# alexrich021/3dvnet

Hardware: AMD Instinct MI355X
Metric: depth maps/sec (256x320, 96 planes, 7 src) (higher is better)
Workload: dtype f32 storage/accumulate; MFMA operands split-bf16x3 (hi*hi+hi*lo+lo*hi, 16 mantissa bits); warp/variance f32 VALU; 1 GPU; cfg2: ScanNet-shape 256x320, 1 ref + 7 src (8 edges/ref), 96 planes, 56x56 plane grid, 32-ch quarter features 64x80; fused warp+variance -> CostRegNet -> soft-argmin depth (rows A1-A6); n_img_per_gpu=71, edges_per_ref=8, parallelism=single GPU, launch=eager, ranks_seen=1

## Files before the change

3dvnet_amd/_lib.py:

```python
import ctypes
import os

import torch

_HERE = os.path.dirname(os.path.abspath(__file__))
LIB_PATH = os.path.join(_HERE, 'lib3dvnet_hip.so')
ABI_VERSION = 9
PRECISION = {'split_bf16': 0, 'fp32': 1}


def precision_code(name):
    try:
        return PRECISION[name]
    except KeyError:
        raise ValueError("precision must be 'split_bf16' or 'fp32', got %r" % (name,))


c_void_p, c_int, c_float, c_double, c_size_t = (ctypes.c_void_p, ctypes.c_int, ctypes.c_float,
                                                ctypes.c_double, ctypes.c_size_t)
c_float_p = ctypes.POINTER(ctypes.c_float)
c_float_pp = ctypes.POINTER(c_float_p)

SIGNATURES = {
    'v3d_version': (c_int, []),
    'v3d_last_error': (ctypes.c_char_p, []),
    'v3d_set_option': (c_int, [ctypes.c_char_p, c_int]),
    'v3d_get_option': (c_int, [ctypes.c_char_p, ctypes.POINTER(c_int)]),
    'v3d_timing_enable': (c_int, [c_int]),
    'v3d_timing_collect': (c_int, [c_int, ctypes.c_char_p, c_int, ctypes.POINTER(c_float),
                                   ctypes.POINTER(c_int)]),
    'v3d_psv_workspace_bytes': (c_size_t, [c_int] * 4),
    'v3d_psv_variance_f32': (c_int, [c_void_p] * 7 + [c_int] * 8 + [c_double] * 2 + [c_int] * 3 +
                             [c_void_p, c_void_p, c_size_t, c_void_p]),
    'v3d_psv_sample_positions_f32': (c_int, [c_void_p] * 6 + [c_int] * 7 + [c_double] * 2 + [c_int] * 3 +
                                     [c_void_p, c_void_p, c_void_p, c_size_t, c_void_p]),
    'v3d_psv_variance_split': (c_int, [c_void_p] * 7 + [c_int] * 8 + [c_double] * 2 + [c_int] * 3 +
                               [c_void_p, c_void_p, c_size_t, c_void_p]),
    'v3d_psv_variance_cl8': (c_int, [c_void_p] * 7 + [c_int] * 8 + [c_double] * 2 + [c_int] * 3 +
                             [c_void_p, c_void_p, c_size_t, c_void_p]),
    'v3d_costreg_depth_cl8': (c_int, [c_void_p] * 3 + [c_int] * 4 + [c_void_p, c_void_p, c_void_p,
                                                                    c_size_t, c_void_p]),
    'v3d_costreg_pack': (c_int, [c_float_pp] * 5 + [c_float_p, c_float_p, c_int, c_int, c_float,
                                                     ctypes.POINTER(c_void_p)]),
    'v3d_costreg_free': (None, [c_void_p]),
    'v3d_costreg_workspace_bytes': (c_size_t, [c_void_p] + [c_int] * 4),
    'v3d_costreg_depth_f32': (c_int, [c_void_p] * 3 + [c_int] * 4 + [c_void_p, c_void_p, c_int, c_void_p,
                                                                    c_size_t, c_void_p]),
    'v3d_costreg_depth_split': (c_int, [c_void_p] * 3 + [c_int] * 4 + [c_void_p, c_void_p, c_void_p,
                                                                      c_size_t, c_void_p]),
    'v3d_costreg_layer_f32': (c_int, [c_void_p, c_int, c_void_p, c_void_p] + [c_int] * 4 +
                              [c_void_p, c_int, c_void_p]),
    'v3d_costreg_layer_split_workspace_bytes': (c_size_t, [c_int] * 5),
    'v3d_costreg_layer_split_f32': (c_int, [c_void_p, c_int, c_void_p, c_void_p] + [c_int] * 4 +
                                    [c_void_p, c_void_p, c_size_t, c_void_p]),
    'v3d_propagation_pack': (c_int, [c_float_pp] * 5 + [c_int, c_int, c_float, ctypes.POINTER(c_void_p)]),
    'v3d_propagation_free': (None, [c_void_p]),
    'v3d_propagation_up_f32': (c_int, [c_void_p, c_void_p, c_void_p] + [c_int] * 6 + [c_void_p, c_void_p, c_void_p, c_int, c_void_p]),
    'v3d_backproject_workspace_bytes': (c_size_t, [c_int] * 4),
    'v3d_backproject_variance_f32': (c_int, [c_void_p] * 8 + [c_int] * 10 + [c_double, c_int] +
                                     [c_void_p, c_void_p, c_void_p, c_size_t, c_void_p]),
    'v3d_gemm_pack': (c_int, [c_float_p, ctypes.c_longlong, ctypes.c_longlong, ctypes.c_longlong,
                              c_int, c_int, c_int, c_float_p, c_float_p, c_float_p, c_float_p,
                              ctypes.POINTER(c_void_p)]),
    'v3d_gemm_free': (None, [c_void_p]),
    'v3d_gemm_gather_f32': (c_int, [c_void_p, c_int, ctypes.POINTER(c_void_p), ctypes.POINTER(c_void_p),
                                    ctypes.POINTER(c_int), c_int, c_int, c_int, c_float, c_void_p, c_int,
                                    c_int, c_void_p, c_void_p, c_int, c_void_p, c_int, c_int, c_void_p]),
    'v3d_sparse_conv_f32': (c_int, [c_void_p, c_int, c_void_p, c_int, c_void_p, ctypes.c_longlong, c_int, c_float, c_void_p,
                                    c_int, c_int, c_void_p, c_int, c_int, c_void_p]),
    'v3d_fill_f32': (c_int, [c_void_p, c_size_t, c_float, c_void_p]),
    'v3d_pointnet_input_f32': (c_int, [c_void_p] * 5 + [c_int, c_int, c_void_p, c_void_p]),
    'v3d_hash_bytes': (c_size_t, [c_int]),
    'v3d_hash_build': (c_int, [c_void_p, c_int, c_void_p, c_size_t, c_void_p]),
    'v3d_hash_status': (c_int, [c_void_p, c_int, c_void_p]),
    'v3d_sparse_neighbors': (c_int, [c_void_p, c_int, c_void_p, c_int, c_int, c_void_p, c_void_p]),
    'v3d_sparse_interp_workspace_bytes': (c_size_t, [c_int, c_int]),
    'v3d_sparse_interp_f32': (c_int, [c_void_p, c_int, c_void_p, c_int, c_int, c_void_p, c_void_p, c_int,
                                      c_int, c_void_p, c_float, c_void_p, c_int, c_int, c_void_p, c_size_t,
                                      c_void_p]),
    'v3d_edges_csr_workspace_bytes': (c_size_t, [c_int, c_int]),
    'v3d_edges_csr': (c_int, [c_void_p, c_int, c_int, c_int, c_void_p, c_void_p, c_void_p, c_void_p, c_size_t, c_void_p]),
    'v3d_edges_csr_status': (c_int, [c_void_p, c_size_t, c_void_p]),
    'v3d_segment_csr_workspace_bytes': (c_size_t, [c_int]),
    'v3d_segment_csr': (c_int, [c_void_p, c_int, c_int, c_void_p, c_void_p, c_void_p, c_size_t, c_void_p]),
    'v3d_segment_max_f32': (c_int, [c_void_p, c_int, c_void_p, c_void_p, c_int, c_int, c_void_p, c_int, c_void_p]),
    'v3d_sort_unique_workspace_bytes': (c_size_t, [c_int]),
    'v3d_sort_unique_u64': (c_int, [c_void_p, c_int, c_void_p, ctypes.POINTER(c_int), c_void_p, c_size_t, c_void_p]),
    'v3d_strided_keys': (c_int, [c_void_p, c_int, c_int, c_void_p, c_void_p]),
    'v3d_unpack_coords': (c_int, [c_void_p, c_int, c_void_p, c_void_p]),
    'v3d_voxelize_workspace_bytes': (c_size_t, []),
    'v3d_voxel_keys': (c_int, [c_void_p, c_void_p, c_int, c_float, c_void_p, c_void_p, c_size_t, c_void_p]),
    'v3d_voxelize_status': (c_int, [c_void_p, c_size_t, c_void_p]),
    'v3d_lower_bound_u64': (c_int, [c_void_p, c_int, c_void_p, c_int, c_void_p, c_void_p]),
    'v3d_voxel_decode': (c_int, [c_void_p, c_int, c_float, c_float, c_void_p, c_void_p, c_void_p, c_void_p,
                                 c_size_t, c_void_p]),
    'v3d_decoder_fused_f32': (c_int, [ctypes.POINTER(c_void_p), c_void_p, c_void_p, ctypes.POINTER(c_void_p),
                                      ctypes.POINTER(c_int), ctypes.POINTER(c_void_p), ctypes.POINTER(c_int),
                                      ctypes.POINTER(c_int), ctypes.POINTER(c_void_p), ctypes.POINTER(c_float), c_void_p,
                                      c_void_p, c_void_p, c_int, c_int, c_int, c_void_p, c_void_p, c_void_p, c_void_p, c_void_p,
                                      c_size_t, c_void_p]),
    'v3d_decoder_fused_workspace_bytes': (c_size_t, [c_int, c_int]),
    'v3d_conv_pack': (c_int, [c_float_p, c_float_p, c_int, c_int, ctypes.POINTER(c_void_p)]),
    'v3d_conv_free': (None, [c_void_p]),
    'v3d_conv_nhwc_f32': (c_int, [c_void_p, c_void_p] + [c_int] * 7 + [c_void_p, c_void_p, c_void_p]),
    'v3d_depthwise_nhwc_f32': (c_int, [c_void_p] * 3 + [c_int] * 7 + [c_void_p, c_void_p]),
    'v3d_stem_f32': (c_int, [c_void_p] * 3 + [c_int] * 3 + [c_void_p, c_void_p]),
    'v3d_nhwc_to_nchw_f32': (c_int, [c_void_p, c_void_p, c_int, c_int, c_int, c_void_p]),
    'v3d_irb_pack': (c_int, [c_float_p] * 6 + [c_int] * 6 + [ctypes.POINTER(c_void_p)]),
    'v3d_irb_free': (None, [c_void_p]),
    'v3d_irb_supported': (c_int, [c_void_p, c_int, c_int]),
    'v3d_irb_workspace_bytes': (c_size_t, [c_void_p, c_int, c_int, c_int]),
    'v3d_stem_block_pack': (c_int, [c_float_p] * 6 + [ctypes.POINTER(c_void_p)]),
    'v3d_stem_block_f32': (c_int, [c_void_p, c_void_p, c_int, c_int, c_int, c_void_p, c_void_p]),
    'v3d_irb_nhwc_f32': (c_int, [c_void_p, c_void_p, c_int, c_int, c_int, c_void_p, c_void_p, c_size_t, c_void_p]),
    'v3d_fpn_pack': (c_int, [c_float_p] * 4 + [c_int, ctypes.POINTER(c_void_p)]),
    'v3d_fpn_free': (None, [c_void_p]),
    'v3d_fpn_level_f32': (c_int, [c_void_p, c_void_p, c_void_p, c_int, c_int, c_int, c_void_p, c_void_p, c_void_p]),
    'v3d_decoder_head_f32': (c_int, [c_void_p, c_int, c_int, c_int, c_void_p, c_void_p, c_void_p, c_void_p,
                                     c_void_p, c_void_p]),
    'v3d_fusion_workspace_bytes': (c_size_t, [c_int] * 3),
    'v3d_fuse_depths_f32': (c_int, [c_void_p, c_void_p, c_int, c_int, c_int, ctypes.POINTER(c_int), c_int, ctypes.POINTER(c_int),
                                    ctypes.POINTER(c_int), c_double, c_void_p, c_void_p, c_void_p, c_size_t, c_void_p]),
    'v3d_fusion_compact': (c_int, [c_void_p, c_void_p, c_void_p] + [c_int] * 5 + [c_void_p] * 7 + [c_size_t, c_void_p]),
    'v3d_cloud_downsample_workspace_bytes': (c_size_t, [c_int]),
    'v3d_cloud_downsample_f32': (c_int, [c_void_p, c_void_p, c_int, c_int, c_void_p, c_double, c_void_p, c_void_p, c_void_p,
                                         c_void_p, c_size_t, c_void_p]),
    'v3d_cloud_status': (c_int, [c_void_p, c_size_t, ctypes.POINTER(c_int), c_void_p]),
    'v3d_nn_workspace_bytes': (c_size_t, [c_int, c_int]),
    'v3d_nn_query_f32': (c_int, [c_void_p, c_int, c_void_p, c_int, c_void_p, c_void_p, c_void_p, c_size_t, c_void_p]),
    'v3d_cloud_metrics_workspace_bytes': (c_size_t, []),
    'v3d_cloud_metrics_f64': (c_int, [c_void_p, c_int, c_void_p, c_int, c_double, c_void_p, c_void_p, c_size_t, c_void_p]),
    'v3d_tsdf_integrate_f32': (c_int, [c_void_p, c_void_p, c_void_p, c_int, c_int, c_int, c_double, c_float_p, c_double, c_void_p,
                                       c_void_p, c_void_p, c_int, c_int, c_int, c_void_p]),
    'v3d_tsdf_normalize_f32': (c_int, [c_void_p, c_void_p, c_void_p, c_int, c_void_p, c_void_p, c_void_p]),
    'v3d_mesh_workspace_bytes': (c_size_t, [c_int, c_int, c_int]),
    'v3d_mesh_count_f32': (c_int, [c_void_p, c_int, c_int, c_int, c_int, c_void_p, c_void_p, c_size_t, c_void_p]),
    'v3d_mesh_extract_f32': (c_int, [c_void_p, c_void_p, c_int, c_int, c_int, c_double, c_float_p, c_int, c_void_p, c_void_p, c_int,
                                     c_void_p, c_int, c_void_p, c_size_t, c_void_p]),
}


class V3DLibraryError(RuntimeError):
    """lib3dvnet_hip.so is missing / unloadable, or a call returned an error code."""


_ERR_NAMES = {-1: 'V3D_ERR_BAD_SHAPE', -2: 'V3D_ERR_BAD_ARG', -3: 'V3D_ERR_WORKSPACE_TOO_SMALL',
              -4: 'V3D_ERR_HIP', -5: 'V3D_ERR_UNSUPPORTED'}
_lib = None


def load():
    global _lib
    if _lib is not None:
        return _lib
    if not os.path.exists(LIB_PATH):
        raise V3DLibraryError('%s not found: the HIP extension is not built (run '
                              '`python 3dvnet_amd/build.py`); there is no CPU fallback' % LIB_PATH)
    try:
        lib = ctypes.CDLL(LIB_PATH)
    except OSError as e:
        raise V3DLibraryError('cannot load %s: %s' % (LIB_PATH, e))
    for name, (res, args) in SIGNATURES.items():
        try:
            fn = getattr(lib, name)
        except AttributeError:
            raise V3DLibraryError('%s does not export %s' % (LIB_PATH, name))
        fn.restype = res
        fn.argtypes = args
    if lib.v3d_version() != ABI_VERSION:
        raise V3DLibraryError('ABI version mismatch: library %d, binding %d'
                              % (lib.v3d_version(), ABI_VERSION))
    _lib = lib
    for item in filter(None, os.environ.get('V3D_OPTIONS', '').split(',')):
        name, _, val = item.partition('=')
        check(lib.v3d_set_option(name.strip().encode(), int(val)), 'v3d_set_option(%s)' % item)
        import warnings
        warnings.warn('3dvnet_amd: developer option %s = %d applied from the V3D_OPTIONS environment variable'
                      % (name.strip(), int(val)), RuntimeWarning, stacklevel=2)
    return lib


def check(rc, what):
    if rc != 0:
        msg = load().v3d_last_error()
        raise V3DLibraryError('%s failed: %s (%s)' % (what, _ERR_NAMES.get(rc, rc),
                                                      msg.decode() if msg else ''))


def set_option(name, value):
    lib = load()
    old = c_int(0)
    check(lib.v3d_get_option(name.encode(), ctypes.byref(old)), 'v3d_get_option')
    check(lib.v3d_set_option(name.encode(), int(value)), 'v3d_set_option')
    return old.value


def ptr(t):
    if t is None:
        return None
    assert t.is_contiguous(), 'tensor passed to the C ABI must be contiguous'
    return t.data_ptr()


def stream_ptr(device):
    return torch.cuda.current_stream(device).cuda_stream


def timing_enable(on=True):
    load().v3d_timing_enable(1 if on else 0)


def timing_collect(max_entries=64):
    lib = load()
    stride = 64
    names = ctypes.create_string_buffer(max_entries * stride)
    ms = (c_float * max_entries)()
    cnt = (c_int * max_entries)()
    n = lib.v3d_timing_collect(max_entries, names, stride, ms, cnt)
    out = {}
    for i in range(n):
        out[names.raw[i * stride:(i + 1) * stride].split(b'\0')[0].decode()] = (float(ms[i]), int(cnt[i]))
    return out
```

3dvnet_amd/build.py:

```python
import glob
import hashlib
import os
import subprocess
import sys

HERE = os.path.dirname(os.path.abspath(__file__))
ROOT = os.path.dirname(HERE)
CSRC = os.path.join(HERE, 'csrc')
LIB = os.path.join(HERE, 'lib3dvnet_hip.so')
HIPCC = os.environ.get('HIPCC', '/opt/rocm/bin/hipcc')
FLAGS = ['--offload-arch=gfx950', '-O3', '-std=c++17', '-fPIC', '-Wall', '-Wno-unused-function',
         '-I', os.path.join(ROOT, 'include'), '-I', CSRC] + os.environ.get('V3D_EXTRA_FLAGS', '').split()


def sources():
    return sorted(glob.glob(os.path.join(CSRC, '*.hip')))


def _flags_tag():
    return hashlib.sha256(' '.join([HIPCC] + FLAGS).encode()).hexdigest()[:12]


def _stale(target, deps):
    if not os.path.exists(target):
        return True
    t = os.path.getmtime(target)
    return any(os.path.getmtime(d) > t for d in deps)


def build(force=False, verbose=False, strict=False):
    headers = glob.glob(os.path.join(CSRC, '*.h')) + glob.glob(os.path.join(ROOT, 'include', '*.h'))
    tag = _flags_tag()
    objdir = os.path.join(HERE, 'build', tag)
    os.makedirs(objdir, exist_ok=True)
    stamp = os.path.join(HERE, 'build', 'linked_flags')
    linked = open(stamp).read().strip() if os.path.exists(stamp) else None
    procs, objs = [], []
    for src in sources():
        obj = os.path.join(objdir, os.path.basename(src)[:-4] + '.o')
        objs.append(obj)
        if force or _stale(obj, [src] + headers):
            cmd = [HIPCC] + FLAGS + ['-c', src, '-o', obj]
            if verbose:
                print(' '.join(cmd))
            procs.append((src, subprocess.Popen(cmd, stdout=subprocess.PIPE, stderr=subprocess.STDOUT)))
    for src, p in procs:
        out, _ = p.communicate()
        if p.returncode != 0:
            sys.stderr.write(out.decode())
            raise RuntimeError('hipcc failed on %s' % src)
        if verbose and out:
            print(out.decode())
    if not os.environ.get('V3D_EXTRA_FLAGS', '').strip() and not os.environ.get('V3D_SKIP_LDS_CHECK'):
        sys.path.insert(0, HERE)
        try:
            import isa_check
            isa_check.check(os.path.join(objdir, 'decoder.o'), strict=strict)
            isa_check.check_wide_lds(os.path.join(objdir, 'irb.o'), 'irb_kernel', strict=strict)
            isa_check.check_wide_lds(os.path.join(objdir, 'fpn.o'), 'fpn_level_kernel', strict=strict)
            isa_check.check_wide_lds(os.path.join(objdir, 'propz.o'), 'propz_kernel', strict=strict)
            isa_check.check_no_scratch(os.path.join(objdir, 'fusion.o'), 'fuse_depths_kernel', strict=strict)
            isa_check.check_no_scratch(os.path.join(objdir, 'tsdf.o'), 'tsdf_integrate_kernel', strict=strict)
            isa_check.check_no_scratch(os.path.join(objdir, 'cloudmetrics.o'), 'nn_query_kernel', strict=strict)
            isa_check.check_no_scratch(os.path.join(objdir, 'mesh.o'), 'mc_[a-z_]*_kernel', strict=strict)
        finally:
            sys.path.pop(0)
    if force or procs or linked != tag or _stale(LIB, objs):
        cmd = [HIPCC, '--offload-arch=gfx950', '-shared', '-fPIC', '-o', LIB] + objs
        if verbose:
            print(' '.join(cmd))
        subprocess.check_call(cmd)
        with open(stamp, 'w') as f:
            f.write(tag + '\n')
    return LIB


if __name__ == '__main__':
    print(build(force='--force' in sys.argv, verbose='--verbose' in sys.argv))
```

3dvnet_amd/csrc/api.hip:

```cpp
#include <atomic>
#include <cstring>
#include <map>
#include <mutex>
#include <string>
#include <vector>

#include "v3d_common.h"

extern "C" int v3d_version(void) { return 9; }

extern "C" const char* v3d_last_error(void) { return v3d::err_buf(); }

namespace {
struct Span { std::string name; hipEvent_t a, b; };
std::mutex g_mu;
bool g_on = false;
std::vector<Span> g_spans;
std::vector<hipEvent_t> g_pool;
hipEvent_t take_event() {
  if (!g_pool.empty()) { hipEvent_t e = g_pool.back(); g_pool.pop_back(); return e; }
  hipEvent_t e; (void)hipEventCreate(&e); return e;
}
}

namespace v3d {
bool timing_enabled() { return g_on; }
void timing_begin(const char* name, hipStream_t s) {
  std::lock_guard<std::mutex> lk(g_mu);
  Span sp{name, take_event(), take_event()};
  (void)hipEventRecord(sp.a, s);
  g_spans.push_back(sp);
}
void timing_end(hipStream_t s) {
  std::lock_guard<std::mutex> lk(g_mu);
  if (!g_spans.empty()) (void)hipEventRecord(g_spans.back().b, s);
}
}

namespace {
struct OptDef { const char* name; int def; };
const OptDef kOptDefs[v3d::kOptCount] = {{"psv_kernel", 0}, {"c12_march", 1}, {"stop_after", 99}, {"gemm_rounds", 1},
                                         {"gemm_pipe", 1}};
std::atomic<int> g_opt[v3d::kOptCount];
std::atomic<bool> g_opt_init{false};
void opt_init() {
  if (!g_opt_init.load(std::memory_order_acquire)) {
    std::lock_guard<std::mutex> lk(g_mu);
    if (!g_opt_init.load()) {
      for (int i = 0; i < v3d::kOptCount; ++i) g_opt[i].store(kOptDefs[i].def);
      g_opt_init.store(true, std::memory_order_release);
    }
  }
}
}

int v3d::option(v3d::Option o) {
  opt_init();
  return g_opt[o].load(std::memory_order_relaxed);
}

extern "C" int v3d_set_option(const char* name, int value) {
  V3D_REQUIRE(name, V3D_ERR_BAD_ARG, "v3d_set_option: null name");
  opt_init();
  for (int i = 0; i < v3d::kOptCount; ++i)
    if (!strcmp(name, kOptDefs[i].name)) {
      V3D_REQUIRE(!(i == v3d::kOptGemmRounds || i == v3d::kOptGemmPipe) || value == 0 || value == 1, V3D_ERR_BAD_ARG,
                  "v3d_set_option: %s must be 0 or 1 (got %d)", name, value);
      g_opt[i].store(value);
      return V3D_OK;
    }
  return v3d::fail(V3D_ERR_BAD_ARG, "v3d_set_option: unknown option '%s'", name);
}

extern "C" int v3d_get_option(const char* name, int* value) {
  V3D_REQUIRE(name && value, V3D_ERR_BAD_ARG, "v3d_get_option: null argument");
  opt_init();
  for (int i = 0; i < v3d::kOptCount; ++i)
    if (!strcmp(name, kOptDefs[i].name)) { *value = g_opt[i].load(); return V3D_OK; }
  return v3d::fail(V3D_ERR_BAD_ARG, "v3d_get_option: unknown option '%s'", name);
}

extern "C" int v3d_timing_enable(int on) {
  std::lock_guard<std::mutex> lk(g_mu);
  g_on = on != 0;
  return V3D_OK;
}

extern "C" int v3d_timing_collect(int max_entries, char* names, int name_stride, float* total_ms,
                                  int* launches) {
  std::lock_guard<std::mutex> lk(g_mu);
  std::map<std::string, std::pair<float, int>> agg;
  std::vector<std::string> order;
  for (auto& sp : g_spans) {
    float ms = 0.f;
    if (hipEventSynchronize(sp.b) == hipSuccess) (void)hipEventElapsedTime(&ms, sp.a, sp.b);
    if (!agg.count(sp.name)) order.push_back(sp.name);
    agg[sp.name].first += ms;
    agg[sp.name].second += 1;
    g_pool.push_back(sp.a);
    g_pool.push_back(sp.b);
  }
  g_spans.clear();
  int n = 0;
  for (auto& k : order) {
    if (n >= max_entries) break;
    if (names && name_stride > 0) {
      strncpy(names + (size_t)n * name_stride, k.c_str(), name_stride - 1);
      names[(size_t)n * name_stride + name_stride - 1] = 0;
    }
    if (total_ms) total_ms[n] = agg[k].first;
    if (launches) launches[n] = agg[k].second;
    ++n;
  }
  return n;
}
```

3dvnet_amd/csrc/psv_variance.hip:

```cpp
#include <cstdlib>

#include <vector>

#include "bf16_split.h"
#include "v3d_common.h"

namespace {

constexpr int kThreads = 256;
constexpr int kPix = 64;
constexpr int kDB = 4;
constexpr int kMaxE = 8;

struct PsvParams {
  const float* featT;
  const float* K;
  const float* R;
  const float* t;
  const int* ref_img;
  const int* edge_ofs;
  const int* edge_src;
  float* var;
  const float* camp;
  int n_img, n_ref, Hf, Wf, H, W, D, h, w, n_ptile;
  double x_step, y_step, z_start, z_step, z_end;
  float rWm1, rHm1;
  unsigned m_dchunk, m_ptile, m_w;
};


template <int C>
__global__ __launch_bounds__(256) void transpose_channel_last_kernel(const float* __restrict__ in,
                                                                      float* __restrict__ out,
                                                                      int HW) {
  __shared__ float tile[C][kPix + 1];
  const int img = blockIdx.y;
  const int p0 = blockIdx.x * kPix;
  const float* src = in + (size_t)img * C * HW;
  float* dst = out + (size_t)img * HW * C;
  for (int i = threadIdx.x; i < C * kPix; i += 256) {
    int c = i / kPix, p = i % kPix;
    tile[c][p] = (p0 + p < HW) ? src[(size_t)c * HW + p0 + p] : 0.f;
  }
  __syncthreads();
  for (int i = threadIdx.x; i < C * kPix; i += 256) {
    int p = i / C, c = i % C;
    if (p0 + p < HW) dst[(size_t)(p0 + p) * C + c] = tile[c][p];
  }
}

__host__ __device__ constexpr int kTailCells(int Wf) { return 2 * (Wf + 2) + 16; }

template <int C>
__global__ __launch_bounds__(256) void transpose_bordered_kernel(const float* __restrict__ in, float* __restrict__ out, int Hf,
                                                                  int Wf, int n_img) {
  __shared__ float tile[C][kPix + 1];
  const int img = blockIdx.y;
  const int Wp = Wf + 2, HW = Hf * Wf, n_cell = (Hf + 2) * Wp;
  const int q0 = blockIdx.x * kPix;
  const float* src = in + (size_t)img * C * HW;
  float* dst = out + (size_t)img * n_cell * C;
  for (int i = threadIdx.x; i < C * kPix; i += 256) {
    const int c = i / kPix, q = q0 + i % kPix;
    const int yb = q / Wp, xb = q - yb * Wp;
    const bool inside = q < n_cell && yb >= 1 && yb <= Hf && xb >= 1 && xb <= Wf;
    tile[c][i % kPix] = inside ? src[(size_t)c * HW + (yb - 1) * Wf + xb - 1] : 0.f;
  }
  __syncthreads();
  for (int i = threadIdx.x; i < C * kPix; i += 256) {
    const int px = i / C, c = i % C;
    if (q0 + px < n_cell) dst[(size_t)(q0 + px) * C + c] = tile[c][px];
  }
  if (img == n_img - 1 && blockIdx.x == 0) {
    float* tail = out + (size_t)n_img * n_cell * C;
    for (int i = threadIdx.x; i < kTailCells(Wf) * C; i += 256) tail[i] = 0.f;
  }
}

#ifdef V3D_PHASE_TIMING
constexpr int kPhaseSlots = 1 << 16;
__device__ unsigned long long g_psv_phase[8 * kPhaseSlots];
#define PHASE_DECL                                  \
  long long ph_t = __builtin_readcyclecounter();    \
  long long ph_acc[8] = {0, 0, 0, 0, 0, 0, 0, 0}
#define PHASE_MARK(i)                                   \
  do {                                                  \
    long long t_ = __builtin_readcyclecounter();        \
    ph_acc[i] += t_ - ph_t;                             \
    ph_t = t_;                                          \
  } while (0)
#define PHASE_FLUSH                                                                                       \
  do {                                                                                                    \
    if (threadIdx.x == 0 && blockIdx.x < kPhaseSlots)                                                     \
      for (int i_ = 0; i_ < 8; ++i_) g_psv_phase[blockIdx.x * 8 + i_] = (unsigned long long)ph_acc[i_];   \
  } while (0)
#else
#define PHASE_DECL
#define PHASE_MARK(i)
#define PHASE_FLUSH
#endif

constexpr int kCamStride = 36;

__global__ void cam_setup_kernel(const float* __restrict__ K, const float* __restrict__ R,
                                 const float* __restrict__ t, float* __restrict__ camp, int n_img) {
  const int img = blockIdx.x * blockDim.x + threadIdx.x;
  if (img >= n_img) return;
  const float* Kp = K + img * 9;
  const float* Rp = R + img * 9;
  const float* tp = t + img * 3;
  float* o = camp + img * kCamStride;
  double a = Kp[0], bb = Kp[1], c = Kp[2], d = Kp[3], e = Kp[4], f = Kp[5], g = Kp[6], hh = Kp[7], i = Kp[8];
  double det = a * (e * i - f * hh) - bb * (d * i - f * g) + c * (d * hh - e * g);
  double id = 1.0 / det;
  o[0] = (float)((e * i - f * hh) * id);
  o[1] = (float)((c * hh - bb * i) * id);
  o[2] = (float)((bb * f - c * e) * id);
  o[3] = (float)((f * g - d * i) * id);
  o[4] = (float)((a * i - c * g) * id);
  o[5] = (float)((c * d - a * f) * id);
  o[6] = (float)((d * hh - e * g) * id);
  o[7] = (float)((bb * g - a * hh) * id);
  o[8] = (float)((a * e - bb * d) * id);
  for (int k = 0; k < 9; ++k) o[9 + k] = Rp[k];
  for (int k = 0; k < 3; ++k) o[18 + k] = tp[k];
  for (int r = 0; r < 3; ++r)
    for (int j = 0; j < 4; ++j) {
      const float b0 = j < 3 ? Rp[0 * 3 + j] : tp[0], b1 = j < 3 ? Rp[1 * 3 + j] : tp[1], b2 = j < 3 ? Rp[2 * 3 + j] : tp[2];
      o[24 + r * 4 + j] = v3d::add_rn(v3d::add_rn(v3d::mul_rn(Kp[r * 3 + 0], b0), v3d::mul_rn(Kp[r * 3 + 1], b1)),
                                    v3d::mul_rn(Kp[r * 3 + 2], b2));
    }
}

struct TapInfo {
  float w00, w01, w10, w11;
  unsigned b00;
  unsigned pad[3];
};

template <unsigned CB>
__device__ __forceinline__ TapInfo make_taps(float ix, float iy, int Wf, int Hf, int first_cell) {
  ix = fminf(fmaxf(ix, -1.f), (float)Wf);
  iy = fminf(fmaxf(iy, -1.f), (float)Hf);
  const float x0 = floorf(ix), y0 = floorf(iy);
  const float x1 = x0 + 1.f, y1 = y0 + 1.f;
  const float wx0 = x1 - ix, wx1 = ix - x0, wy0 = y1 - iy, wy1 = iy - y0;
  TapInfo ti;
  ti.w00 = v3d::mul_rn(wx0, wy0); ti.w01 = v3d::mul_rn(wx1, wy0);
  ti.w10 = v3d::mul_rn(wx0, wy1); ti.w11 = v3d::mul_rn(wx1, wy1);
  ti.b00 = (unsigned)(first_cell + ((int)y0 + 1) * (Wf + 2) + (int)x0 + 1) * CB;
  return ti;
}

typedef float f32x4 __attribute__((ext_vector_type(4)));
typedef unsigned int u32x2 __attribute__((ext_vector_type(2)));
typedef unsigned int u32x4 __attribute__((ext_vector_type(4)));

using v3d::bf16_rne;
using v3d::pack_bf16x2;

template <int C, bool SPLIT>
__global__ __launch_bounds__(64) void psv_variance_kernel(PsvParams p) {
  constexpr int kThreads = 64, kPix = kThreads / 4;
  constexpr int LP = C / 4;
  constexpr int PPP = kThreads / LP;
  constexpr int NPASS = kPix / PPP;
  static_assert(kPix % PPP == 0, "tile");

  __shared__ TapInfo s_tap[kMaxE * kPix];
  __shared__ __attribute__((aligned(16))) float s_out[C][kPix + 1];
  __shared__ float s_ref[24];
  __shared__ float s_P[kMaxE][12];

  const int tid = threadIdx.x;
  const int n_dchunk = (p.D + kDB - 1) / kDB;
  int b = v3d::xcd_contiguous_block();
  const int ptile = b % p.n_ptile; b /= p.n_ptile;
  const int dchunk = b % n_dchunk;
  const int r = b / n_dchunk;
  const int P = p.h * p.w;
  const int e_begin = p.edge_ofs[r], e_end = p.edge_ofs[r + 1];
  const int ne = e_end - e_begin;
  const int ref = p.ref_img[r];

  if (tid < 21) s_ref[tid] = p.camp[ref * kCamStride + tid];

  const int cg = tid % LP;
  const int pix_in_pass = tid / LP;

  const int px1 = tid % kPix;
  const int gp1 = ptile * kPix + px1;
  float xf = 0.f, yf = 0.f;
  {
    int gy = gp1 / p.w, gx = gp1 % p.w;
    xf = (p.w > 1 && gx == p.w - 1) ? (float)(p.W - 1) : (float)((double)gx * p.x_step);
    yf = (p.h > 1 && gy == p.h - 1) ? (float)(p.H - 1) : (float)((double)gy * p.y_step);
  }
  const float Wm1 = (float)(p.W - 1), Hm1 = (float)(p.H - 1);
  const float rWm1 = (float)(1.0 / (double)(p.W - 1)), rHm1 = (float)(1.0 / (double)(p.H - 1));
  const float Wfm1 = (float)(p.Wf - 1), Hfm1 = (float)(p.Hf - 1);

  PHASE_DECL;
  for (int dd = 0; dd < kDB; ++dd) {
    const int d = dchunk * kDB + dd;
    if (d >= p.D) break;
    const float z = (d == p.D - 1 && p.D > 1) ? (float)p.z_end
                                               : (float)(p.z_start + (double)d * p.z_step);
    float acc_s[NPASS][4], acc_q[NPASS][4];
#pragma unroll
    for (int a = 0; a < NPASS; ++a)
#pragma unroll
      for (int k = 0; k < 4; ++k) acc_s[a][k] = acc_q[a][k] = 0.f;

    for (int ec = 0; ec < ne; ec += kMaxE) {
      const int nec = min(kMaxE, ne - ec);
      __syncthreads();
      PHASE_MARK(0);
      if (dd == 0 || ne > kMaxE) {
        for (int i = tid; i < nec * 12; i += kThreads)
          s_P[i / 12][i % 12] = p.camp[p.edge_src[e_begin + ec + i / 12] * kCamStride + 24 + i % 12];
      }
      __syncthreads();
      PHASE_MARK(1);
      {
        float X, Y, Z;
        v3d::world_point(s_ref, xf, yf, z, X, Y, Z);
        for (int e = tid / kPix; e < nec; e += kThreads / kPix) {
          float ix, iy;
          v3d::sample_position(s_P[e], X, Y, Z, Wm1, rWm1, Hm1, rHm1, Wfm1, Hfm1, ix, iy);
          const TapInfo ti = make_taps<4 * C>(ix, iy, p.Wf, p.Hf, p.edge_src[e_begin + ec + e] * (p.Hf + 2) * (p.Wf + 2));
          s_tap[e * kPix + px1] = ti;
        }
      }
      PHASE_MARK(2);
      __syncthreads();
      PHASE_MARK(3);
#pragma unroll
      for (int a = 0; a < NPASS; ++a) {
        const int px = a * PPP + pix_in_pass;
        for (int e = 0; e < nec; ++e) {
          const TapInfo ti = s_tap[e * kPix + px];
          float4 s;
          {
            const char* fb = reinterpret_cast<const char*>(p.featT);
            const unsigned cgb = cg * 16, rowb = (unsigned)(p.Wf + 2) * (4 * C);
            const float4 v00 = *reinterpret_cast<const float4*>(fb + (size_t)(ti.b00 + cgb));
            const float4 v01 = *reinterpret_cast<const float4*>(fb + (size_t)(ti.b00 + cgb) + 4 * C);
            const float4 v10 = *reinterpret_cast<const float4*>(fb + (size_t)(ti.b00 + rowb + cgb));
            const float4 v11 = *reinterpret_cast<const float4*>(fb + (size_t)(ti.b00 + rowb + cgb) + 4 * C);
            s.x = v3d::mul_rn(v00.x, ti.w00); s.y = v3d::mul_rn(v00.y, ti.w00);
            s.z = v3d::mul_rn(v00.z, ti.w00); s.w = v3d::mul_rn(v00.w, ti.w00);
            s.x = __builtin_fmaf(v01.x, ti.w01, s.x); s.y = __builtin_fmaf(v01.y, ti.w01, s.y);
            s.z = __builtin_fmaf(v01.z, ti.w01, s.z); s.w = __builtin_fmaf(v01.w, ti.w01, s.w);
            s.x = __builtin_fmaf(v10.x, ti.w10, s.x); s.y = __builtin_fmaf(v10.y, ti.w10, s.y);
            s.z = __builtin_fmaf(v10.z, ti.w10, s.z); s.w = __builtin_fmaf(v10.w, ti.w10, s.w);
            s.x = __builtin_fmaf(v11.x, ti.w11, s.x); s.y = __builtin_fmaf(v11.y, ti.w11, s.y);
            s.z = __builtin_fmaf(v11.z, ti.w11, s.z); s.w = __builtin_fmaf(v11.w, ti.w11, s.w);
          }
          acc_s[a][0] = v3d::add_rn(acc_s[a][0], s.x); acc_s[a][1] = v3d::add_rn(acc_s[a][1], s.y);
          acc_s[a][2] = v3d::add_rn(acc_s[a][2], s.z); acc_s[a][3] = v3d::add_rn(acc_s[a][3], s.w);
          acc_q[a][0] = __builtin_fmaf(s.x, s.x, acc_q[a][0]); acc_q[a][1] = __builtin_fmaf(s.y, s.y, acc_q[a][1]);
          acc_q[a][2] = __builtin_fmaf(s.z, s.z, acc_q[a][2]); acc_q[a][3] = __builtin_fmaf(s.w, s.w, acc_q[a][3]);
        }
      }
    }
    PHASE_MARK(4);
    const float cnt = (float)max(ne, 1);
    if constexpr (SPLIT) {
      static_assert(!SPLIT || C == 32, "split layout is defined for 32 channels");
      u32x2* const s_sp = reinterpret_cast<u32x2*>(&s_out[0][0]);
      const int chunk = cg >> 1, half = cg & 1;
#pragma unroll
      for (int a = 0; a < NPASS; ++a) {
        const int px = a * PPP + pix_in_pass;
        unsigned h[4], l[4];
#pragma unroll
        for (int k = 0; k < 4; ++k) {
          const float avg = acc_s[a][k] / cnt;
          const float avg_sq = acc_q[a][k] / cnt;
          const float v = v3d::sub_rn(avg_sq, v3d::mul_rn(avg, avg));
          h[k] = bf16_rne(v);
          l[k] = bf16_rne(v - __uint_as_float(h[k] << 16));
        }
        s_sp[(((chunk * 2 + 0) * (kPix + 1)) + px) * 2 + half] = (u32x2){h[0] | (h[1] << 16), h[2] | (h[3] << 16)};
        s_sp[(((chunk * 2 + 1) * (kPix + 1)) + px) * 2 + half] = (u32x2){l[0] | (l[1] << 16), l[2] | (l[3] << 16)};
      }
      __syncthreads();
      u32x4* const out = reinterpret_cast<u32x4*>(p.var);
      const u32x4* const s_q = reinterpret_cast<const u32x4*>(s_sp);
      for (int i = tid; i < 8 * kPix; i += kThreads) {
        const int g = i / kPix, px = i % kPix;
        const int gp = ptile * kPix + px;
        if (gp < P) __builtin_nontemporal_store(s_q[g * (kPix + 1) + px], &out[(((size_t)r * 8 + g) * p.D + d) * P + gp]);
      }
    } else {
#pragma unroll
      for (int a = 0; a < NPASS; ++a) {
        const int px = a * PPP + pix_in_pass;
#pragma unroll
        for (int k = 0; k < 4; ++k) {
          float avg = acc_s[a][k] / cnt;
          float avg_sq = acc_q[a][k] / cnt;
          s_out[cg * 4 + k][px] = v3d::sub_rn(avg_sq, v3d::mul_rn(avg, avg));
        }
      }
      __syncthreads();
      {
        const int px = tid % kPix;
        const int gp = ptile * kPix + px;
        if (gp < P) {
          for (int c = tid / kPix; c < C; c += kThreads / kPix)
            __builtin_nontemporal_store(s_out[c][px], &p.var[(((size_t)r * C + c) * p.D + d) * P + gp]);
        }
      }
    }
    PHASE_MARK(5);
  }
  PHASE_FLUSH;
}


constexpr int kRPix = 8;
#ifndef V3D_PSV_RDB
#define V3D_PSV_RDB 8
#endif
constexpr int kRDB = V3D_PSV_RDB;
constexpr int kRE = 64 / (kRDB * kRPix);

#ifndef V3D_PSV_WAVES
#define V3D_PSV_WAVES 4
#endif
#ifndef V3D_PSV_ABLATE
#define V3D_PSV_ABLATE 0
#endif
template <int WPB>
__device__ __forceinline__ void psv_wave_sync() {
  if constexpr (WPB == 1) __syncthreads();
  else { __builtin_amdgcn_fence(__ATOMIC_SEQ_CST, "workgroup"); __builtin_amdgcn_wave_barrier(); }
}

template <bool SPLIT>
__global__ __launch_bounds__(SPLIT ? 64 : 256, V3D_PSV_WAVES) void psv_variance_reuse_kernel(PsvParams p) {
  constexpr int C = 32, WPB = SPLIT ? 1 : 4;
  constexpr int kOutPl = 4;
  static_assert(SPLIT || kRDB % kOutPl == 0, "fp32 epilogue stages 4 planes per round");
  __shared__ TapInfo s_tap_[WPB][kRE * kRDB * kRPix];
  __shared__ __attribute__((aligned(16))) float s_out[SPLIT ? 1 : kOutPl][SPLIT ? 1 : C][SPLIT ? 1 : WPB * kRPix + 1];
  __shared__ float s_ref_[WPB][24];
  __shared__ float s_P_[WPB][kMaxE][12];
  __shared__ int s_base_[WPB][kMaxE];

  const int lane = threadIdx.x & 63;
  const int wv = __builtin_amdgcn_readfirstlane(threadIdx.x >> 6);
  TapInfo* const s_tap = s_tap_[wv];
  float* const s_ref = s_ref_[wv];
  float (*const s_P)[12] = s_P_[wv];
  int* const s_base = s_base_[wv];
  const int n_dchunk = (p.D + kRDB - 1) / kRDB;
  int b = v3d::xcd_contiguous_block();
  const int dchunk = b % n_dchunk; b /= n_dchunk;
  const int ptile = (b % p.n_ptile) * WPB + wv;
  const int r = b / p.n_ptile;
  const int P = p.h * p.w;
  const int e_begin = p.edge_ofs[r], e_end = p.edge_ofs[r + 1];
  const int ne = e_end - e_begin;
  const int ref = p.ref_img[r];
  if (lane < 21) s_ref[lane] = p.camp[ref * kCamStride + lane];
  psv_wave_sync<WPB>();

  const int e1 = lane / (kRDB * kRPix), pl1 = (lane >> 3) & (kRDB - 1), px1 = lane & 7;
  const int gp1 = ptile * kRPix + px1;
  const int d1 = dchunk * kRDB + pl1;
  float X, Y, Z;
  {
    const int gy = gp1 / p.w, gx = gp1 % p.w;
    const float xf = (p.w > 1 && gx == p.w - 1) ? (float)(p.W - 1) : (float)((double)gx * p.x_step);
    const float yf = (p.h > 1 && gy == p.h - 1) ? (float)(p.H - 1) : (float)((double)gy * p.y_step);
    const float z = (d1 == p.D - 1 && p.D > 1) ? (float)p.z_end : (float)(p.z_start + (double)d1 * p.z_step);
    v3d::world_point(s_ref, xf, yf, z, X, Y, Z);
  }
  const bool live1 = gp1 < P && d1 < p.D;
  const float Wm1 = (float)(p.W - 1), Hm1 = (float)(p.H - 1);
  const float rWm1 = (float)(1.0 / (double)(p.W - 1)), rHm1 = (float)(1.0 / (double)(p.H - 1));
  const float Wfm1 = (float)(p.Wf - 1), Hfm1 = (float)(p.Hf - 1);

  const int gpx = lane >> 3;
  const unsigned cgb = (lane & 7) * 16;
  const unsigned rowb = (unsigned)(p.Wf + 2) * (4 * C) + cgb;
  const char* const fb = reinterpret_cast<const char*>(p.featT);
  f32x4 acc_s[kRDB], acc_q[kRDB];
#pragma unroll
  for (int k = 0; k < kRDB; ++k) acc_s[k] = acc_q[k] = (f32x4){0.f, 0.f, 0.f, 0.f};

  PHASE_DECL;
  for (int ec = 0; ec < ne; ec += kRE) {
    const int nec = min(kRE, ne - ec);
    psv_wave_sync<WPB>();
    PHASE_MARK(0);
    if (ec % kMaxE == 0) {
      const int nload = min(kMaxE, ne - ec) * 12;
#pragma unroll 1
      for (int i = lane; i < nload; i += 64) {
        const int src = p.edge_src[e_begin + ec + i / 12];
        s_P[i / 12][i % 12] = p.camp[src * kCamStride + 24 + i % 12];
        if (i % 12 == 0) s_base[i / 12] = src * (p.Hf + 2) * (p.Wf + 2);
      }
      psv_wave_sync<WPB>();
    }
#if V3D_PSV_ABLATE == 3
    if (ec == 0)
#endif
    if (e1 < nec) {
      float ix, iy;
      v3d::sample_position(s_P[ec % kMaxE + e1], X, Y, Z, Wm1, rWm1, Hm1, rHm1, Wfm1, Hfm1, ix, iy);
      s_tap[(e1 * kRDB + pl1) * kRPix + px1] = make_taps<4 * C>(ix, iy, p.Wf, p.Hf, s_base[ec % kMaxE + e1]);
    }
    psv_wave_sync<WPB>();
    PHASE_MARK(1);
    for (int e = 0; e < nec; ++e) {
      unsigned c00 = ~0u;
      f32x4 t00, t01, t10, t11;
#pragma unroll
      for (int pl = 0; pl < kRDB; ++pl) {
        const TapInfo ti = s_tap[(e * kRDB + pl) * kRPix + gpx];
#if V3D_PSV_ABLATE == 2
        if (pl == 0) {
#else
        if (ti.b00 != c00) {
#endif
          t00 = *reinterpret_cast<const f32x4*>(fb + (size_t)(ti.b00 + cgb));
          t01 = *reinterpret_cast<const f32x4*>(fb + (size_t)(ti.b00 + cgb) + 4 * C);
          t10 = *reinterpret_cast<const f32x4*>(fb + (size_t)(ti.b00 + rowb));
          t11 = *reinterpret_cast<const f32x4*>(fb + (size_t)(ti.b00 + rowb) + 4 * C);
          c00 = ti.b00;
        }
#if V3D_PSV_ABLATE == 1
        asm volatile("" : : "v"(t00), "v"(t01), "v"(t10), "v"(t11), "v"(ti.w00), "v"(ti.w01), "v"(ti.w10), "v"(ti.w11));
#else
        f32x4 sv = t00 * ti.w00;
        sv = __builtin_elementwise_fma(t01, (f32x4){ti.w01, ti.w01, ti.w01, ti.w01}, sv);
        sv = __builtin_elementwise_fma(t10, (f32x4){ti.w10, ti.w10, ti.w10, ti.w10}, sv);
        sv = __builtin_elementwise_fma(t11, (f32x4){ti.w11, ti.w11, ti.w11, ti.w11}, sv);
        acc_s[pl] += sv;
        acc_q[pl] = __builtin_elementwise_fma(sv, sv, acc_q[pl]);
#endif
#ifndef V3D_PSV_NOSERIAL
        asm volatile("" : "+v"(acc_s[pl]), "+v"(acc_q[pl]) : : "memory");
#endif
      }
    }
    PHASE_MARK(4);
  }

  PHASE_MARK(2);
  psv_wave_sync<WPB>();
  const float cnt = (float)max(ne, 1);
  const bool cnt_pow2 = (max(ne, 1) & (max(ne, 1) - 1)) == 0;
  const float cnt_inv = 1.f / cnt;
#ifdef V3D_PSV_EXACT_DIV
  auto mean = [&](float x) __attribute__((always_inline)) { return x / cnt; };
#else
  auto mean = [&](float x) __attribute__((always_inline)) { return cnt_pow2 ? x * cnt_inv : x / cnt; };
#endif
  const int cg = lane & 7;
  if constexpr (SPLIT) {
    const int chunk = cg >> 1, half = cg & 1;
    u32x4* const out = reinterpret_cast<u32x4*>(p.var);
    const int gp = ptile * kRPix + gpx;
#pragma unroll
    for (int pl = 0; pl < kRDB; ++pl) {
      float v[4];
#pragma unroll
      for (int k = 0; k < 4; ++k) {
        const float avg = mean(acc_s[pl][k]);
        const float avg_sq = mean(acc_q[pl][k]);
        v[k] = v3d::sub_rn(avg_sq, v3d::mul_rn(avg, avg));
      }
      const unsigned h01 = pack_bf16x2(v[0], v[1]), h23 = pack_bf16x2(v[2], v[3]);
      const unsigned l01 = pack_bf16x2(v[0] - __uint_as_float(h01 << 16), v[1] - __uint_as_float(h01 & 0xffff0000u));
      const unsigned l23 = pack_bf16x2(v[2] - __uint_as_float(h23 << 16), v[3] - __uint_as_float(h23 & 0xffff0000u));
      const unsigned s0 = half ? h01 : l01, s1 = half ? h23 : l23;
      const unsigned r0 = (unsigned)__builtin_amdgcn_mov_dpp((int)s0, 0xB1, 0xf, 0xf, true);
      const unsigned r1 = (unsigned)__builtin_amdgcn_mov_dpp((int)s1, 0xB1, 0xf, 0xf, true);
      const u32x4 slot = half ? (u32x4){r0, r1, l01, l23} : (u32x4){h01, h23, r0, r1};
      const int d = dchunk * kRDB + pl;
      if (gp < P && d < p.D && (V3D_PSV_ABLATE != 4 || slot[0] == 0x12345u))
#ifdef V3D_PSV_PLAIN_STORE
        out[(((size_t)r * 8 + chunk * 2 + half) * p.D + d) * P + gp] = slot;
#else
        __builtin_nontemporal_store(slot, &out[(((size_t)r * 8 + chunk * 2 + half) * p.D + d) * P + gp]);
#endif
    }
  } else {
    constexpr int NPX = WPB * kRPix;
    const int gp0 = (ptile - wv) * kRPix;
#pragma unroll
    for (int round = 0; round < kRDB / kOutPl; ++round) {
      if (round) __syncthreads();
#pragma unroll
      for (int q = 0; q < kOutPl; ++q) {
        const int pl = round * kOutPl + q;
#pragma unroll
        for (int k = 0; k < 4; ++k) {
          const float avg = mean(acc_s[pl][k]);
          const float avg_sq = mean(acc_q[pl][k]);
          s_out[q][cg * 4 + k][wv * kRPix + gpx] = v3d::sub_rn(avg_sq, v3d::mul_rn(avg, avg));
        }
      }
      __syncthreads();
      for (int i = threadIdx.x; i < kOutPl * C * NPX; i += 64 * WPB) {
        const int q = i / (C * NPX), c = (i / NPX) % C, px = i % NPX;
        const int gp = gp0 + px, d = dchunk * kRDB + round * kOutPl + q;
        if (gp < P && d < p.D) __builtin_nontemporal_store(s_out[q][c][px], &p.var[(((size_t)r * C + c) * p.D + d) * P + gp]);
      }
    }
  }
  PHASE_MARK(3);
  PHASE_FLUSH;
}

constexpr int kWinCols = 16, kWinRows = 4;
typedef float psv_f32x2 __attribute__((ext_vector_type(2)));

__device__ __forceinline__ int psv_smin(int a, int b) { int r; asm("s_min_i32 %0, %1, %2" : "=s"(r) : "s"(a), "s"(b) : "scc"); return r; }
__device__ __forceinline__ int psv_smax(int a, int b) { int r; asm("s_max_i32 %0, %1, %2" : "=s"(r) : "s"(a), "s"(b) : "scc"); return r; }

#ifndef V3D_PSVW_ABLATE
#define V3D_PSVW_ABLATE 0
#endif
template <bool SPLIT, bool CL8 = false>
__global__ __launch_bounds__(SPLIT ? 64 : 256, V3D_PSV_WAVES) void psv_variance_window_kernel(PsvParams p) {
  static_assert(SPLIT || !CL8, "the channel-last fp32 output uses the single-wave geometry");
  constexpr int C = 32, WPB = SPLIT ? 1 : 4;
  constexpr unsigned CB = 4 * C;
  constexpr int kOutPl = 4;
  static_assert(kWinCols == 16 && kRDB == 8 && kRE == 1, "the window kernel projects one edge per pass: 8 planes x 8 pixels = 64 lanes");
  __shared__ __attribute__((aligned(16))) float s_win_[WPB][kWinRows * kWinCols * C];
  __shared__ __attribute__((aligned(16))) f32x4 s_w_[WPB][kRDB * kRPix];
  __shared__ unsigned s_slot_[WPB][kRDB * kRPix];
  __shared__ float s_ref_[WPB][24];
  __shared__ float s_P_[WPB][kMaxE][12];
  __shared__ int s_base_[WPB][kMaxE];
  static_assert(SPLIT || kOutPl * C * (WPB * kRPix + 1) <= WPB * kWinRows * kWinCols * C, "epilogue staging fits the windows");

  const int lane = threadIdx.x & 63;
  const int wv = __builtin_amdgcn_readfirstlane(threadIdx.x >> 6);
  float* const s_win = s_win_[wv];
  f32x4* const s_w = s_w_[wv];
  unsigned* const s_slot = s_slot_[wv];
  float* const s_ref = s_ref_[wv];
  float (*const s_P)[12] = s_P_[wv];
  int* const s_base = s_base_[wv];
  const int n_dchunk = (p.D + kRDB - 1) / kRDB;
  const unsigned b = (unsigned)v3d::xcd_contiguous_block();
  const unsigned b1 = v3d::udiv_magic(b, (unsigned)n_dchunk, p.m_dchunk), b2 = v3d::udiv_magic(b1, (unsigned)p.n_ptile, p.m_ptile);
  const int dchunk = (int)(b - b1 * (unsigned)n_dchunk);
  const int ptile = (int)(b1 - b2 * (unsigned)p.n_ptile) * WPB + wv;
  const int r = (int)b2;
  const int P = p.h * p.w;
  const int e_begin = p.edge_ofs[r], e_end = p.edge_ofs[r + 1];
  const int ne = e_end - e_begin;
  const int ref = p.ref_img[r];
  if (lane < 21) s_ref[lane] = p.camp[ref * kCamStride + lane];
  psv_wave_sync<WPB>();

  const int pl1 = lane >> 3, px1 = lane & 7;
  const int gp1 = ptile * kRPix + px1;
  const int d1 = dchunk * kRDB + pl1;
  float X, Y, Z;
  {
    int gy, gx;
    if (p.w >= kRPix) {
      const unsigned g0 = (unsigned)(ptile * kRPix), gy0 = v3d::udiv_magic(g0, (unsigned)p.w, p.m_w);
      gx = (int)(g0 - gy0 * (unsigned)p.w) + px1;
      gy = (int)gy0;
      if (gx >= p.w) { gx -= p.w; ++gy; }
    } else {
      gy = gp1 / p.w; gx = gp1 % p.w;
    }
    const float xf = (p.w > 1 && gx == p.w - 1) ? (float)(p.W - 1) : (float)((double)gx * p.x_step);
    const float yf = (p.h > 1 && gy == p.h - 1) ? (float)(p.H - 1) : (float)((double)gy * p.y_step);
    const float z = (d1 == p.D - 1 && p.D > 1) ? (float)p.z_end : (float)(p.z_start + (double)d1 * p.z_step);
    v3d::world_point(s_ref, xf, yf, z, X, Y, Z);
  }
  const bool live1 = gp1 < P && d1 < p.D;
  const bool all_live = __all(live1);
  const float Wm1 = (float)(p.W - 1), Hm1 = (float)(p.H - 1);
  const float rWm1 = p.rWm1, rHm1 = p.rHm1;
  const float Wfm1 = (float)(p.Wf - 1), Hfm1 = (float)(p.Hf - 1);
  const int Wp = p.Wf + 2;
  const float Wff = (float)p.Wf, Hff = (float)p.Hf;

  const int gpx = lane >> 3;
  const unsigned cgb = (lane & 7) * 16;
  const unsigned rowb = (unsigned)Wp * CB + cgb;
  const unsigned lane16 = (unsigned)lane * 16u;
  const char* const fb = reinterpret_cast<const char*>(p.featT);
  const char* const wb = reinterpret_cast<const char*>(s_win);
  const unsigned win_lds = __builtin_amdgcn_readfirstlane(
      (unsigned)(size_t)(__attribute__((address_space(3))) void*)s_win);
  f32x4 acc_s[kRDB], acc_q[kRDB];
#pragma unroll
  for (int k = 0; k < kRDB; ++k) acc_s[k] = acc_q[k] = (f32x4){0.f, 0.f, 0.f, 0.f};

#if V3D_PSVW_ABLATE == 1
#define V3D_PSV_BLEND(pl_, w_) asm volatile("" : : "v"(t00), "v"(t01), "v"(t10), "v"(t11), "v"(w_) : "memory")
#else
#define V3D_PSV_BLEND(pl_, w_)                                                                       \
  do {                                                                                               \
    f32x4 sv_ = t00 * (w_)[0];                                                                       \
    sv_ = __builtin_elementwise_fma(t01, (f32x4){(w_)[1], (w_)[1], (w_)[1], (w_)[1]}, sv_);          \
    sv_ = __builtin_elementwise_fma(t10, (f32x4){(w_)[2], (w_)[2], (w_)[2], (w_)[2]}, sv_);          \
     \
    {                                                                                                \
      psv_f32x2 lo_ = {sv_[0], sv_[1]}, hi_ = {sv_[2], sv_[3]};                                      \
      const psv_f32x2 w23_ = {(w_)[2], (w_)[3]};                                                     \
      const psv_f32x2 tl_ = {t11[0], t11[1]}, th_ = {t11[2], t11[3]};                                \
      asm("v_pk_fma_f32 %0, %1, %2, %0 op_sel:[0,1,0] op_sel_hi:[1,1,1]" : "+v"(lo_) : "v"(tl_), "v"(w23_));  \
      asm("v_pk_fma_f32 %0, %1, %2, %0 op_sel:[0,1,0] op_sel_hi:[1,1,1]" : "+v"(hi_) : "v"(th_), "v"(w23_));  \
      sv_ = (f32x4){lo_[0], lo_[1], hi_[0], hi_[1]};                                                 \
    }                                                                                                \
    acc_s[pl_] += sv_;                                                                               \
    acc_q[pl_] = __builtin_elementwise_fma(sv_, sv_, acc_q[pl_]);                                    \
                            \
    asm volatile("" : "+v"(acc_s[pl_]), "+v"(acc_q[pl_]) : : "memory");                              \
  } while (0)
#endif

  auto load_cams = [&](int e0) __attribute__((always_inline)) {
    const int nload = min(kMaxE, ne - e0) * 12;
#pragma unroll 1
    for (int i = lane; i < nload; i += 64) {
      const int src = p.edge_src[e_begin + e0 + i / 12];
      s_P[i / 12][i % 12] = p.camp[src * kCamStride + 24 + i % 12];
      if (i % 12 == 0) s_base[i / 12] = src * (p.Hf + 2) * Wp;
    }
  };
  auto project = [&](int e, int& xb, int& yb, f32x4& wq) __attribute__((always_inline)) {
    float ix, iy;
    v3d::sample_position(s_P[e % kMaxE], X, Y, Z, Wm1, rWm1, Hm1, rHm1, Wfm1, Hfm1, ix, iy);
    ix = __builtin_amdgcn_fmed3f(ix, -1.f, Wff);
    iy = __builtin_amdgcn_fmed3f(iy, -1.f, Hff);
    const float x0 = floorf(ix), y0 = floorf(iy);
    const float x1 = x0 + 1.f, y1 = y0 + 1.f;
    const float wx0 = x1 - ix, wx1 = ix - x0, wy0 = y1 - iy, wy1 = iy - y0;
    wq = (f32x4){v3d::mul_rn(wx0, wy0), v3d::mul_rn(wx1, wy0), v3d::mul_rn(wx0, wy1), v3d::mul_rn(wx1, wy1)};
    xb = (int)x0 + 1;
    yb = (int)y0 + 1;
    if (!all_live) {
      const int xb0 = __builtin_amdgcn_readlane(xb, 0), yb0 = __builtin_amdgcn_readlane(yb, 0);
      xb = live1 ? xb : xb0;
      yb = live1 ? yb : yb0;
    }
  };
  int xb = 0, yb = 0;
  f32x4 wq = {0.f, 0.f, 0.f, 0.f};
  if (ne > 0) {
    load_cams(0);
    psv_wave_sync<WPB>();
    project(0, xb, yb, wq);
  }
  for (int e = 0; e < ne; ++e) {
    psv_wave_sync<WPB>();
#ifdef V3D_PSV_NOPIPE
    if (e > 0) {
      if (e % kMaxE == 0) { load_cams(e); psv_wave_sync<WPB>(); }
      project(e, xb, yb, wq);
    }
#endif
    int xmin, ymin, ncol, nrow;
    {
      const int cc = (yb << 16) | xb;
      const int ca = __builtin_amdgcn_readlane(cc, 0), cb = __builtin_amdgcn_readlane(cc, 7);
      const int cd = __builtin_amdgcn_readlane(cc, 56), ce = __builtin_amdgcn_readlane(cc, 63);
      const int xa = ca & 0xffff, xc = cb & 0xffff, xd = cd & 0xffff, xe = ce & 0xffff;
      const int ya = ca >> 16, yc = cb >> 16, yd = cd >> 16, ye = ce >> 16;
      xmin = psv_smin(psv_smin(xa, xc), psv_smin(xd, xe));
      ymin = psv_smin(psv_smin(ya, yc), psv_smin(yd, ye));
      ncol = psv_smax(psv_smax(xa, xc), psv_smax(xd, xe)) - xmin + 2 > 8 ? kWinCols : 8;
      nrow = psv_smin(psv_smax(psv_smax(ya, yc), psv_smax(yd, ye)) - ymin + 2, kWinRows);
    }
    const int base_cell = __builtin_amdgcn_readfirstlane(s_base[e % kMaxE]);
    const unsigned dx = (unsigned)(xb - xmin), dy = (unsigned)(yb - ymin);
    const bool inwin = dx <= (unsigned)(ncol - 2) && dy <= (unsigned)(nrow - 2);
    const unsigned so_win = ((dy << 4) | dx) * CB;
    const unsigned so_ext = ((unsigned)(base_cell + __mul24(yb, Wp) + xb) * CB) | 0x80000000u;
    const unsigned so = inwin ? so_win : so_ext;
    s_w[lane] = wq;
    s_slot[lane] = so;
    const unsigned prev = (unsigned)__builtin_amdgcn_ds_bpermute(((lane - 8) & 63) * 4, (int)so);
    const unsigned long long chg = __ballot(lane < 8 || so != prev);
    {
      const char* rowp = fb + (size_t)((unsigned)(base_cell + ymin * Wp + xmin) * CB);
      unsigned dst = win_lds;
      asm volatile("s_nop 4" ::: "memory");
#pragma unroll 1
      for (int rr = 0; rr < (V3D_PSVW_ABLATE == 3 ? 0 : nrow); ++rr) {
        unsigned keep;
        asm volatile("s_mov_b32 %0, m0\n\ts_mov_b32 m0, %3\n\ts_nop 0\n\tglobal_load_lds_dwordx4 %1, %2\n\ts_mov_b32 m0, %0"
                     : "=&s"(keep) : "v"(lane16), "s"(rowp), "s"(dst) : "memory");
        if (ncol > 8)
          asm volatile("s_mov_b32 %0, m0\n\ts_mov_b32 m0, %3\n\ts_nop 0\n\tglobal_load_lds_dwordx4 %1, %2 offset:1024\n\ts_mov_b32 m0, %0"
                       : "=&s"(keep) : "v"(lane16), "s"(rowp), "s"(dst) : "memory");
        rowp += (size_t)Wp * CB;
        dst += kWinCols * CB;
      }
    }
#ifndef V3D_PSV_NOPIPE
    if (e + 1 < ne) {
      if ((e + 1) % kMaxE == 0) {
        psv_wave_sync<WPB>();
        load_cams(e + 1);
        psv_wave_sync<WPB>();
      }
      project(e + 1, xb, yb, wq);
    }
#endif
    asm volatile("s_waitcnt vmcnt(0) lgkmcnt(0)" ::: "memory");
    psv_wave_sync<WPB>();
    f32x4 t00, t01, t10, t11;
    f32x4 wn = s_w[gpx];
    unsigned sn = s_slot[gpx];
#pragma unroll
    for (int pl = 0; pl < kRDB; ++pl) {
      const f32x4 w = wn;
      const unsigned so_pl = sn;
      if (pl + 1 < kRDB) {
        wn = s_w[(pl + 1) * kRPix + gpx];
        sn = s_slot[(pl + 1) * kRPix + gpx];
      }
      if (((chg >> (8 * pl)) & 0xffull) && (V3D_PSVW_ABLATE != 2 || (pl == 0 && e == 0))) {
        if (V3D_PSVW_ABLATE != 6 && (int)so_pl < 0) {
          const unsigned b00 = so_pl & 0x7fffffffu;
          t00 = *reinterpret_cast<const f32x4*>(fb + (size_t)(b00 + cgb));
          t01 = *reinterpret_cast<const f32x4*>(fb + (size_t)(b00 + cgb) + CB);
          t10 = *reinterpret_cast<const f32x4*>(fb + (size_t)(b00 + rowb));
          t11 = *reinterpret_cast<const f32x4*>(fb + (size_t)(b00 + rowb) + CB);
        } else {
          const char* a = wb + (so_pl + cgb);
          t00 = *reinterpret_cast<const f32x4*>(a);
          t01 = *reinterpret_cast<const f32x4*>(a + CB);
          t10 = *reinterpret_cast<const f32x4*>(a + kWinCols * CB);
          t11 = *reinterpret_cast<const f32x4*>(a + kWinCols * CB + CB);
        }
      }
      V3D_PSV_BLEND(pl, w);
    }
  }
#undef V3D_PSV_BLEND

  psv_wave_sync<WPB>();
  const float cnt = (float)max(ne, 1);
  const bool cnt_pow2 = (max(ne, 1) & (max(ne, 1) - 1)) == 0;
  const float cnt_inv = 1.f / cnt;
  const int cg = lane & 7;
  if constexpr (SPLIT) {
    const int chunk = cg >> 1, half = cg & 1;
    u32x4* const out = reinterpret_cast<u32x4*>(p.var);
    const int gp = ptile * kRPix + gpx;
    u32x4* const obase = out + (((size_t)r * 8 + chunk * 2 + half) * p.D + (size_t)dchunk * kRDB) * P + gp;
#define V3D_PSV_EMIT(MEAN)                                                                                              \
  _Pragma("unroll") for (int pl = 0; pl < kRDB; ++pl) {                                                                 \
    float v[4];                                                                                                         \
    _Pragma("unroll") for (int k = 0; k < 4; ++k) {                                                                     \
      const float avg = MEAN(acc_s[pl][k]);                                                                             \
      const float avg_sq = MEAN(acc_q[pl][k]);                                                                          \
      v[k] = v3d::sub_rn(avg_sq, v3d::mul_rn(avg, avg));                                             \
    }                                                                                                                   \
    const int d = dchunk * kRDB + pl;                                                                                   \
    if constexpr (CL8) {                                                                                                \
               \
      const u32x4 slot = {__float_as_uint(v[0]), __float_as_uint(v[1]), __float_as_uint(v[2]), __float_as_uint(v[3])};  \
      if (gp < P && d < p.D)                                                                                            \
        __builtin_nontemporal_store(slot, obase + (size_t)pl * (unsigned)P);                                             \
    } else {                                                                                                            \
    const unsigned h01 = pack_bf16x2(v[0], v[1]), h23 = pack_bf16x2(v[2], v[3]);                                        \
    const unsigned l01 = pack_bf16x2(v[0] - __uint_as_float(h01 << 16), v[1] - __uint_as_float(h01 & 0xffff0000u));     \
    const unsigned l23 = pack_bf16x2(v[2] - __uint_as_float(h23 << 16), v[3] - __uint_as_float(h23 & 0xffff0000u));     \
    const unsigned s0 = half ? h01 : l01, s1 = half ? h23 : l23;                       \
    const unsigned r0 = (unsigned)__builtin_amdgcn_mov_dpp((int)s0, 0xB1, 0xf, 0xf, true);      \
    const unsigned r1 = (unsigned)__builtin_amdgcn_mov_dpp((int)s1, 0xB1, 0xf, 0xf, true);                              \
    const u32x4 slot = half ? (u32x4){r0, r1, l01, l23} : (u32x4){h01, h23, r0, r1};                                    \
    if (gp < P && d < p.D && (V3D_PSVW_ABLATE != 5 || slot[0] == 0x12345u))                                             \
      __builtin_nontemporal_store(slot, obase + (size_t)pl * (unsigned)P);                                               \
    }                                                                                                                   \
  }
#define V3D_MEAN_MUL(x) ((x) * cnt_inv)
#define V3D_MEAN_DIV(x) __builtin_amdgcn_div_fixupf(v3d::div_uniform((x), cnt, cnt_inv), cnt, (x))
    if (cnt_pow2) { V3D_PSV_EMIT(V3D_MEAN_MUL) } else { V3D_PSV_EMIT(V3D_MEAN_DIV) }
#undef V3D_PSV_EMIT
#undef V3D_MEAN_MUL
#undef V3D_MEAN_DIV
  } else {
    constexpr int NPX = WPB * kRPix;
    float (*const s_out)[C][NPX + 1] = reinterpret_cast<float (*)[C][NPX + 1]>(&s_win_[0][0]);
    auto mean = [&](float x) __attribute__((always_inline)) {
      return cnt_pow2 ? x * cnt_inv : __builtin_amdgcn_div_fixupf(v3d::div_uniform(x, cnt, cnt_inv), cnt, x);
    };
    const int gp0 = (ptile - wv) * kRPix;
#pragma unroll
    for (int round = 0; round < kRDB / kOutPl; ++round) {
      __syncthreads();
#pragma unroll
      for (int q = 0; q < kOutPl; ++q) {
        const int pl = round * kOutPl + q;
#pragma unroll
        for (int k = 0; k < 4; ++k) {
          const float avg = mean(acc_s[pl][k]);
          const float avg_sq = mean(acc_q[pl][k]);
          s_out[q][cg * 4 + k][wv * kRPix + gpx] = v3d::sub_rn(avg_sq, v3d::mul_rn(avg, avg));
        }
      }
      __syncthreads();
      for (int i = threadIdx.x; i < kOutPl * C * NPX; i += 64 * WPB) {
        const int q = i / (C * NPX), c = (i / NPX) % C, px = i % NPX;
        const int gp = gp0 + px, d = dchunk * kRDB + round * kOutPl + q;
        if (gp < P && d < p.D) __builtin_nontemporal_store(s_out[q][c][px], &p.var[(((size_t)r * C + c) * p.D + d) * P + gp]);
      }
    }
  }
}

__global__ __launch_bounds__(256) void psv_positions_kernel(PsvParams p, float* __restrict__ pos, float* __restrict__ world) {
  const int P = p.h * p.w;
  const long long n_vox = (long long)p.D * P;
  const long long i = (long long)blockIdx.x * 256 + threadIdx.x;
  const int r = blockIdx.y;
  if (i >= n_vox) return;
  const int d = (int)(i / P), gp = (int)(i % P), gy = gp / p.w, gx = gp % p.w;
  const float xf = (p.w > 1 && gx == p.w - 1) ? (float)(p.W - 1) : (float)((double)gx * p.x_step);
  const float yf = (p.h > 1 && gy == p.h - 1) ? (float)(p.H - 1) : (float)((double)gy * p.y_step);
  const float z = (d == p.D - 1 && p.D > 1) ? (float)p.z_end : (float)(p.z_start + (double)d * p.z_step);
  float X, Y, Z;
  v3d::world_point(p.camp + p.ref_img[r] * kCamStride, xf, yf, z, X, Y, Z);
  if (world) {
    world[((size_t)r * 3 + 0) * n_vox + i] = X;
    world[((size_t)r * 3 + 1) * n_vox + i] = Y;
    world[((size_t)r * 3 + 2) * n_vox + i] = Z;
  }
  const float Wm1 = (float)(p.W - 1), Hm1 = (float)(p.H - 1);
  const float rWm1 = (float)(1.0 / (double)(p.W - 1)), rHm1 = (float)(1.0 / (double)(p.H - 1));
  const float Wfm1 = (float)(p.Wf - 1), Hfm1 = (float)(p.Hf - 1);
  for (int e = p.edge_ofs[r]; e < p.edge_ofs[r + 1]; ++e) {
    float ix, iy;
    v3d::sample_position(p.camp + p.edge_src[e] * kCamStride + 24, X, Y, Z, Wm1, rWm1, Hm1, rHm1, Wfm1, Hfm1, ix, iy);
    pos[((size_t)e * n_vox + i) * 2] = ix;
    pos[((size_t)e * n_vox + i) * 2 + 1] = iy;
  }
}

}

int v3d::transpose_channel_last(const float* feat, float* featT, int n_img, int C, int HW, hipStream_t s) {
  dim3 tg((HW + kPix - 1) / kPix, n_img);
  v3d::TimedScope ts("transpose_channel_last", s);
  if (C == 32) transpose_channel_last_kernel<32><<<tg, 256, 0, s>>>(feat, featT, HW);
  else if (C == 16) transpose_channel_last_kernel<16><<<tg, 256, 0, s>>>(feat, featT, HW);
  else return -1;
  return 0;
}

static size_t psv_feat_bytes(int n_img, int C, int Hf, int Wf) {
  return ((size_t)n_img * (Hf + 2) * (Wf + 2) + kTailCells(Wf)) * C * sizeof(float);
}

extern "C" size_t v3d_psv_workspace_bytes(int n_img, int C, int Hf, int Wf) {
  return v3d::align_up(psv_feat_bytes(n_img, C, Hf, Wf), 256) + v3d::align_up((size_t)n_img * kCamStride * sizeof(float), 256);
}

static int psv_variance_impl(int mode, const float* feat, const float* K, const float* R,
                                    const float* t, const int32_t* ref_img,
                                    const int32_t* edge_ofs, const int32_t* edge_src, int n_img,
                                    int n_ref, int n_edges, int C, int Hf, int Wf, int H, int W,
                                    double depth_start, double depth_interval, int D, int h, int w,
                                    float* var, void* workspace, size_t workspace_bytes,
                                    void* stream) {
  const bool split = mode != 0, cl8 = mode == 2;
  V3D_REQUIRE(feat && K && R && t && ref_img && edge_ofs && edge_src && var && workspace,
              V3D_ERR_BAD_ARG, "v3d_psv_variance_f32: null pointer argument");
  V3D_REQUIRE(C == 32 || C == 16, V3D_ERR_UNSUPPORTED,
              "v3d_psv_variance_f32: C=%d unsupported (16 or 32)", C);
  V3D_REQUIRE(W <= (1 << 20) && H <= (1 << 20), V3D_ERR_BAD_SHAPE, "v3d_psv_variance_f32: image size out of range");
  V3D_REQUIRE(!split || C == 32, V3D_ERR_UNSUPPORTED,
              "v3d_psv_variance_split: C=%d unsupported (the split layout is defined for 32 channels)", C);
  V3D_REQUIRE(n_img > 0 && n_ref > 0 && n_edges >= 0 && Hf > 0 && Wf > 0 && H > 1 && W > 1 &&
                  D > 0 && h > 0 && w > 0,
              V3D_ERR_BAD_SHAPE, "v3d_psv_variance_f32: bad shape");
  V3D_REQUIRE(Hf < 32760 && Wf < 32760, V3D_ERR_BAD_SHAPE, "v3d_psv_variance_f32: feature maps larger than 32759 cells per axis");
  V3D_REQUIRE(psv_feat_bytes(n_img, C, Hf, Wf) < (size_t)1 << 32, V3D_ERR_BAD_SHAPE,
              "v3d_psv_variance_f32: bordered feature maps exceed 4 GB (32-bit byte offsets)");
  V3D_REQUIRE(workspace_bytes >= v3d_psv_workspace_bytes(n_img, C, Hf, Wf),
              V3D_ERR_WORKSPACE_TOO_SMALL, "v3d_psv_variance_f32: workspace %zu < %zu",
              workspace_bytes, v3d_psv_workspace_bytes(n_img, C, Hf, Wf));
  hipStream_t s = (hipStream_t)stream;
  float* featT = (float*)workspace;
  float* camp = (float*)((char*)workspace + v3d::align_up(psv_feat_bytes(n_img, C, Hf, Wf), 256));
  {
    v3d::TimedScope ts("transpose_channel_last", s);
    const dim3 tg(((Hf + 2) * (Wf + 2) + kPix - 1) / kPix, n_img);
    if (C == 32) transpose_bordered_kernel<32><<<tg, 256, 0, s>>>(feat, featT, Hf, Wf, n_img);
    else transpose_bordered_kernel<16><<<tg, 256, 0, s>>>(feat, featT, Hf, Wf, n_img);
  }
  V3D_CHECK_LAUNCH("transpose_bordered_kernel");
  cam_setup_kernel<<<(n_img + 63) / 64, 64, 0, s>>>(K, R, t, camp, n_img);
  V3D_CHECK_LAUNCH("cam_setup_kernel");

  PsvParams p;
  p.featT = featT; p.K = K; p.R = R; p.t = t;
  p.ref_img = ref_img; p.edge_ofs = edge_ofs; p.edge_src = edge_src; p.var = var; p.camp = camp;
  p.n_img = n_img; p.n_ref = n_ref; p.Hf = Hf; p.Wf = Wf; p.H = H; p.W = W; p.D = D;
  p.h = h; p.w = w;
  p.n_ptile = (h * w + 15) / 16;
  p.x_step = w > 1 ? (double)(W - 1) / (double)(w - 1) : 0.0;
  p.y_step = h > 1 ? (double)(H - 1) / (double)(h - 1) : 0.0;
  const double depth_end = depth_start + (double)(D - 1) * depth_interval;
  p.z_start = depth_start;
  p.z_step = D > 1 ? (depth_end - depth_start) / (double)(D - 1) : 0.0;
  p.z_end = depth_end;
  const int n_dchunk = (D + kDB - 1) / kDB;
  const long long blocks = (long long)n_ref * n_dchunk * p.n_ptile;
  V3D_REQUIRE(blocks < (1ll << 31), V3D_ERR_BAD_SHAPE, "v3d_psv_variance_f32: grid too large");
  {
    v3d::TimedScope ts("psv_variance", s);
    const unsigned grid = (unsigned)blocks;
    const int psv_kernel = v3d::option(v3d::kOptPsvKernel);
    const bool plain_gather = psv_kernel == 2;
    if (C == 32 && !plain_gather) {
      const long long rblocks = (long long)n_ref * ((D + kRDB - 1) / kRDB) * ((h * w + kRPix - 1) / kRPix);
      V3D_REQUIRE(rblocks < (1ll << 31), V3D_ERR_BAD_SHAPE, "v3d_psv_variance_f32: grid too large");
      p.n_ptile = (h * w + kRPix - 1) / kRPix;
      const bool reuse_env = psv_kernel == 1 || kRDB != 8;
      const bool no_window = reuse_env || psv_feat_bytes(n_img, C, Hf, Wf) >= ((size_t)1 << 31);
      V3D_REQUIRE(!cl8 || !no_window, V3D_ERR_UNSUPPORTED,
                  "v3d_psv_variance_cl8: only the window kernel writes this layout (feature maps < 2 GB, no developer switch)");
      {
        const unsigned ndc = (unsigned)((D + kRDB - 1) / kRDB);
        const unsigned npt = (unsigned)(split || cl8 ? p.n_ptile : (p.n_ptile + 3) / 4);
        const unsigned long long nblk = (unsigned long long)n_ref * ndc * npt;
        p.rWm1 = (float)(1.0 / (double)(W - 1));
        p.rHm1 = (float)(1.0 / (double)(H - 1));
        p.m_dchunk = v3d::magic_u32(nblk, ndc);
        p.m_ptile = v3d::magic_u32(nblk / ndc + 1, npt);
        p.m_w = v3d::magic_u32((unsigned long long)h * w + 4 * kRPix, (unsigned)w);
      }
      if (cl8) {
        psv_variance_window_kernel<true, true><<<(unsigned)rblocks, 64, 0, s>>>(p);
      } else if (split) {
        if (no_window) psv_variance_reuse_kernel<true><<<(unsigned)rblocks, 64, 0, s>>>(p);
        else psv_variance_window_kernel<true><<<(unsigned)rblocks, 64, 0, s>>>(p);
      } else {
        p.n_ptile = (p.n_ptile + 3) / 4;
        const long long fblocks = (long long)n_ref * ((D + kRDB - 1) / kRDB) * p.n_ptile;
        if (no_window) psv_variance_reuse_kernel<false><<<(unsigned)fblocks, 256, 0, s>>>(p);
        else psv_variance_window_kernel<false><<<(unsigned)fblocks, 256, 0, s>>>(p);
      }
    } else if (cl8) {
      return v3d::fail(V3D_ERR_UNSUPPORTED, "v3d_psv_variance_cl8: C=%d unsupported (32) / option psv_kernel = 2", C);
    } else if (split) psv_variance_kernel<32, true><<<grid, 64, 0, s>>>(p);
    else if (C == 32) psv_variance_kernel<32, false><<<grid, 64, 0, s>>>(p);
    else psv_variance_kernel<16, false><<<grid, 64, 0, s>>>(p);
  }
  V3D_CHECK_LAUNCH("psv_variance_kernel");
  return V3D_OK;
}

extern "C" int v3d_psv_sample_positions_f32(const float* K, const float* R, const float* t, const int32_t* ref_img,
                                            const int32_t* edge_ofs, const int32_t* edge_src, int n_img, int n_ref,
                                            int n_edges, int Hf, int Wf, int H, int W, double depth_start,
                                            double depth_interval, int D, int h, int w, float* pos, float* world,
                                            void* workspace, size_t workspace_bytes, void* stream) {
  V3D_REQUIRE(K && R && t && ref_img && edge_ofs && edge_src && pos && workspace, V3D_ERR_BAD_ARG,
              "v3d_psv_sample_positions_f32: null pointer argument");
  V3D_REQUIRE(n_img > 0 && n_ref > 0 && n_edges >= 0 && Hf > 0 && Wf > 0 && H > 1 && W > 1 && D > 0 && h > 0 && w > 0,
              V3D_ERR_BAD_SHAPE, "v3d_psv_sample_positions_f32: bad shape");
  V3D_REQUIRE(workspace_bytes >= (size_t)n_img * kCamStride * sizeof(float), V3D_ERR_WORKSPACE_TOO_SMALL,
              "v3d_psv_sample_positions_f32: workspace too small (n_img * 36 floats)");
  hipStream_t s = (hipStream_t)stream;
  float* camp = (float*)workspace;
  cam_setup_kernel<<<(n_img + 63) / 64, 64, 0, s>>>(K, R, t, camp, n_img);
  PsvParams p;
  memset(&p, 0, sizeof(p));
  p.ref_img = ref_img; p.edge_ofs = edge_ofs; p.edge_src = edge_src; p.camp = camp;
  p.n_img = n_img; p.n_ref = n_ref; p.Hf = Hf; p.Wf = Wf; p.H = H; p.W = W; p.D = D; p.h = h; p.w = w;
  p.x_step = w > 1 ? (double)(W - 1) / (double)(w - 1) : 0.0;
  p.y_step = h > 1 ? (double)(H - 1) / (double)(h - 1) : 0.0;
  const double depth_end = depth_start + (double)(D - 1) * depth_interval;
  p.z_start = depth_start;
  p.z_step = D > 1 ? (depth_end - depth_start) / (double)(D - 1) : 0.0;
  p.z_end = depth_end;
  const long long n_vox = (long long)D * h * w;
  psv_positions_kernel<<<dim3((unsigned)((n_vox + 255) / 256), n_ref), 256, 0, s>>>(p, pos, world);
  V3D_CHECK_LAUNCH("psv_positions_kernel");
  return V3D_OK;
}

extern "C" int v3d_psv_variance_f32(const float* feat, const float* K, const float* R, const float* t,
                                    const int32_t* ref_img, const int32_t* edge_ofs, const int32_t* edge_src,
                                    int n_img, int n_ref, int n_edges, int C, int Hf, int Wf, int H, int W,
                                    double depth_start, double depth_interval, int D, int h, int w, float* var,
                                    void* workspace, size_t workspace_bytes, void* stream) {
  return psv_variance_impl(0, feat, K, R, t, ref_img, edge_ofs, edge_src, n_img, n_ref, n_edges, C, Hf, Wf, H, W,
                           depth_start, depth_interval, D, h, w, var, workspace, workspace_bytes, stream);
}

extern "C" int v3d_psv_variance_split(const float* feat, const float* K, const float* R, const float* t,
                                      const int32_t* ref_img, const int32_t* edge_ofs, const int32_t* edge_src,
                                      int n_img, int n_ref, int n_edges, int C, int Hf, int Wf, int H, int W,
                                      double depth_start, double depth_interval, int D, int h, int w,
                                      void* var_split, void* workspace, size_t workspace_bytes, void* stream) {
  return psv_variance_impl(1, feat, K, R, t, ref_img, edge_ofs, edge_src, n_img, n_ref, n_edges, C, Hf, Wf, H, W,
                           depth_start, depth_interval, D, h, w, (float*)var_split, workspace, workspace_bytes,
                           stream);
}

extern "C" int v3d_psv_variance_cl8(const float* feat, const float* K, const float* R, const float* t,
                                    const int32_t* ref_img, const int32_t* edge_ofs, const int32_t* edge_src,
                                    int n_img, int n_ref, int n_edges, int C, int Hf, int Wf, int H, int W,
                                    double depth_start, double depth_interval, int D, int h, int w,
                                    float* var_cl8, void* workspace, size_t workspace_bytes, void* stream) {
  return psv_variance_impl(2, feat, K, R, t, ref_img, edge_ofs, edge_src, n_img, n_ref, n_edges, C, Hf, Wf, H, W,
                           depth_start, depth_interval, D, h, w, var_cl8, workspace, workspace_bytes, stream);
}

#ifdef V3D_PHASE_TIMING
extern "C" int v3d_debug_psv_phase_read(unsigned long long* out8_host, int n_blocks) {
  V3D_CHECK_HIP(hipDeviceSynchronize());
  std::vector<unsigned long long> h((size_t)8 * kPhaseSlots);
  V3D_CHECK_HIP(hipMemcpyFromSymbol(h.data(), HIP_SYMBOL(g_psv_phase), h.size() * sizeof(unsigned long long)));
  for (int i = 0; i < 8; ++i) out8_host[i] = 0;
  for (int b = 0; b < n_blocks && b < kPhaseSlots; ++b)
    for (int i = 0; i < 8; ++i) out8_host[i] += h[(size_t)b * 8 + i];
  return V3D_OK;
}
#endif
```

3dvnet_amd/csrc/v3d_common.h:

```cpp
#pragma once
#include <hip/hip_runtime.h>

#include <cstdarg>
#include <cstdio>
#include <cstring>

#include "v3d.h"

namespace v3d {

inline char* err_buf() {
  static thread_local char buf[512] = {0};
  return buf;
}

inline int fail(int code, const char* fmt, ...) {
  va_list ap;
  va_start(ap, fmt);
  vsnprintf(err_buf(), 512, fmt, ap);
  va_end(ap);
  return code;
}

#define V3D_CHECK_HIP(expr)                                                                    \
  do {                                                                                         \
    hipError_t e_ = (expr);                                                                    \
    if (e_ != hipSuccess)                                                                      \
      return v3d::fail(V3D_ERR_HIP, "%s failed: %s (%s:%d)", #expr, hipGetErrorString(e_),     \
                       __FILE__, __LINE__);                                                    \
  } while (0)

#define V3D_CHECK_LAUNCH(name)                                                                 \
  do {                                                                                         \
    hipError_t e_ = hipGetLastError();                                                         \
    if (e_ != hipSuccess)                                                                      \
      return v3d::fail(V3D_ERR_HIP, "launch of %s failed: %s", name, hipGetErrorString(e_));   \
  } while (0)

#define V3D_REQUIRE(cond, code, ...)                                                           \
  do {                                                                                         \
    if (!(cond)) return v3d::fail(code, __VA_ARGS__);                                          \
  } while (0)

inline size_t align_up(size_t x, size_t a) { return (x + a - 1) / a * a; }

enum Option {
  kOptPsvKernel,
  kOptC12March,
  kOptStopAfter,
  kOptGemmRounds,
  kOptGemmPipe,
  kOptCount
};
int option(Option o);

bool timing_enabled();
void timing_begin(const char* name, hipStream_t s);
void timing_end(hipStream_t s);

inline unsigned persistent_grid(long long n_tiles, int wgs_per_cu) {
  static int n_cu = 0;
  if (n_cu == 0) {
    int dev = 0, v = 0;
    if (hipGetDevice(&dev) != hipSuccess || hipDeviceGetAttribute(&v, hipDeviceAttributeMultiprocessorCount, dev) != hipSuccess || v <= 0) v = 256;
    n_cu = v;
  }
  long long g = (long long)n_cu * wgs_per_cu;
  if (g > n_tiles) g = n_tiles;
  g = (g + 7) / 8 * 8;
  return (unsigned)g;
}

inline int opt_in_dynamic_lds(const void* kernel, int bytes, bool* done_per_device) {
  int dev = 0;
  V3D_CHECK_HIP(hipGetDevice(&dev));
  V3D_REQUIRE(dev >= 0 && dev < 64, V3D_ERR_UNSUPPORTED, "device ordinal %d", dev);
  if (!done_per_device[dev]) {
    V3D_CHECK_HIP(hipFuncSetAttribute(kernel, hipFuncAttributeMaxDynamicSharedMemorySize, bytes));
    done_per_device[dev] = true;
  }
  return V3D_OK;
}

struct TimedScope {
  hipStream_t s;
  bool on;
  TimedScope(const char* name, hipStream_t s_) : s(s_), on(timing_enabled()) {
    if (on) timing_begin(name, s);
  }
  ~TimedScope() {
    if (on) timing_end(s);
  }
};

__device__ __forceinline__ int xcd_contiguous_block() {
  const int total = (int)gridDim.x, per = total >> 3, rem = total & 7;
  const int x = (int)blockIdx.x & 7, i = (int)blockIdx.x >> 3;
  return x * per + (x < rem ? x : rem) + i;
}

inline unsigned magic_u32(unsigned long long x_max, unsigned d) {
  if (d <= 1 || x_max * d >= (1ull << 32)) return 0u;
  return (unsigned)(((1ull << 32) + d - 1) / d);
}
__device__ __forceinline__ unsigned udiv_magic(unsigned x, unsigned d, unsigned m) { return m ? __umulhi(x, m) : x / d; }

template <int D>
__device__ __forceinline__ unsigned small_div(unsigned x) {
  static_assert(D >= 2 && D < 1024, "small_div: divisor range");
  return __umul24(x, (unsigned)((1 << 20) / D + 1)) >> 20;
}

struct TileWalk { int t, end, step; };
__device__ __forceinline__ TileWalk xcd_tile_walk(int n_tiles) {
  const int G = (int)gridDim.x >> 3;
  const int x = (int)blockIdx.x & 7, i = (int)blockIdx.x >> 3;
  const int per = n_tiles >> 3, rem = n_tiles & 7;
  const int first = x * per + (x < rem ? x : rem);
  return {first + i, first + per + (x < rem ? 1 : 0), G};
}

__device__ __forceinline__ float mul_rn(float a, float b) {
#pragma clang fp contract(off)
  return a * b;
}
__device__ __forceinline__ float add_rn(float a, float b) {
#pragma clang fp contract(off)
  return a + b;
}
__device__ __forceinline__ float sub_rn(float a, float b) {
#pragma clang fp contract(off)
  return a - b;
}

__device__ __forceinline__ float dot3_chain(float a0, float b0, float a1, float b1, float a2, float b2) {
  return __builtin_fmaf(a2, b2, __builtin_fmaf(a1, b1, mul_rn(a0, b0)));
}
__device__ __forceinline__ float dot4h_chain(float a0, float b0, float a1, float b1, float a2, float b2, float a3) {
  return add_rn(dot3_chain(a0, b0, a1, b1, a2, b2), a3);
}

__device__ __forceinline__ void world_point(const float* cam, float xf, float yf, float z, float& X, float& Y, float& Z) {
  const float p0 = mul_rn(xf, z), p1 = mul_rn(yf, z), p2 = z;
  const float c0 = sub_rn(dot3_chain(cam[0], p0, cam[1], p1, cam[2], p2), cam[18]);
  const float c1 = sub_rn(dot3_chain(cam[3], p0, cam[4], p1, cam[5], p2), cam[19]);
  const float c2 = sub_rn(dot3_chain(cam[6], p0, cam[7], p1, cam[8], p2), cam[20]);
  X = dot3_chain(cam[9], c0, cam[12], c1, cam[15], c2);
  Y = dot3_chain(cam[10], c0, cam[13], c1, cam[16], c2);
  Z = dot3_chain(cam[11], c0, cam[14], c1, cam[17], c2);
}

__device__ __forceinline__ float div_uniform(float x, float c, float rc) {
  const float q0 = mul_rn(x, rc);
  return __builtin_fmaf(__builtin_fmaf(-q0, c, x), rc, q0);
}

__device__ __forceinline__ void div2_shared(float x, float y, float den, float& qx, float& qy) {
  float r = __builtin_amdgcn_rcpf(den);
  r = __builtin_fmaf(__builtin_fmaf(-den, r, 1.f), r, r);
  float q = mul_rn(x, r);
  q = __builtin_fmaf(__builtin_fmaf(-den, q, x), r, q);
  q = __builtin_fmaf(__builtin_fmaf(-den, q, x), r, q);
  qx = __builtin_amdgcn_div_fixupf(q, den, x);
  q = mul_rn(y, r);
  q = __builtin_fmaf(__builtin_fmaf(-den, q, y), r, q);
  q = __builtin_fmaf(__builtin_fmaf(-den, q, y), r, q);
  qy = __builtin_amdgcn_div_fixupf(q, den, y);
}

__device__ __forceinline__ void sample_position(const float* Pm, float X, float Y, float Z, float Wm1, float rWm1, float Hm1,
                                                float rHm1, float Wfm1, float Hfm1, float& ix, float& iy) {
  const float qx = dot4h_chain(Pm[0], X, Pm[1], Y, Pm[2], Z, Pm[3]);
  const float qy = dot4h_chain(Pm[4], X, Pm[5], Y, Pm[6], Z, Pm[7]);
  const float qz = dot4h_chain(Pm[8], X, Pm[9], Y, Pm[10], Z, Pm[11]);
  const float zb = add_rn(fabsf(qz), 1e-8f);
  float u, v;
  div2_shared(qx, qy, zb, u, v);
  const float gx = __builtin_fmaf(div_uniform(u, Wm1, rWm1), 2.f, -1.f);
  const float gy = __builtin_fmaf(div_uniform(v, Hm1, rHm1), 2.f, -1.f);
  ix = mul_rn(add_rn(gx, 1.f), mul_rn(0.5f, Wfm1));
  iy = mul_rn(add_rn(gy, 1.f), mul_rn(0.5f, Hfm1));
}

int launch_conv0z(bool f32, const void* in, const float* wimg, const float* bias, void* out, int n, int D, int H, int W,
                  hipStream_t s);

int launch_conv12z(const void* c0_split, const float* w1, const float* w2, const float* b1, const float* b2, void* out_split,
                   int n, int D, int H, int W, hipStream_t s);

int transpose_channel_last(const float* feat, float* featT, int n_img, int C, int HW, hipStream_t s);

}
```

3dvnet_amd/synthetic.py:

```python
import math

import numpy as np
import torch

ROOM = (6.03, 5.01, 2.97)
SCANNET_K = (577.87, 577.87, 319.5, 239.5, 640, 480)


def intrinsics(img_size):
    fx, fy, cx, cy, w0, h0 = SCANNET_K
    sy, sx = img_size[0] / h0, img_size[1] / w0
    return torch.tensor([[fx * sx, 0.0, cx * sx], [0.0, fy * sy, cy * sy], [0.0, 0.0, 1.0]],
                        dtype=torch.float32)


def _rot(axis, ang):
    axis = axis / np.linalg.norm(axis)
    k = np.array([[0, -axis[2], axis[1]], [axis[2], 0, -axis[0]], [-axis[1], axis[0], 0]])
    return np.eye(3) + math.sin(ang) * k + (1 - math.cos(ang)) * (k @ k)


def make_cameras(n_img, img_size, seed=0, yaw_step_deg=None, radius=0.8, height=1.5):
    rng = np.random.RandomState(seed)
    if yaw_step_deg is None:
        yaw_step_deg = min(360.0 / n_img, 6.0)
    cx, cy = ROOM[0] / 2, ROOM[1] / 2
    rotmats, tvecs = [], []
    for i in range(n_img):
        th = math.radians(yaw_step_deg * i)
        f = np.array([math.cos(th), math.sin(th), 0.0])
        d = np.array([0.0, 0.0, -1.0])
        r = np.cross(d, f)
        R_c2w = np.stack([r, d, f], axis=1)
        jit = rng.normal(0, math.radians(0.5), 3)
        for a, ang in zip(np.eye(3), jit):
            R_c2w = _rot(a, ang) @ R_c2w
        c = np.array([cx + radius * math.cos(th), cy + radius * math.sin(th), height])
        c = c + rng.normal(0, 0.01, 3)
        R = R_c2w.T
        rotmats.append(R)
        tvecs.append(-R @ c)
    rotmats = torch.from_numpy(np.stack(rotmats)).float()
    tvecs = torch.from_numpy(np.stack(tvecs)).float()
    K = intrinsics(img_size).unsqueeze(0).repeat(n_img, 1, 1)
    return rotmats, tvecs, K


def make_edges(n_ref, n_before, n_after):
    per = n_before + n_after + 1
    e = torch.empty((2, n_ref * per), dtype=torch.long)
    for i in range(n_ref):
        e[0, i * per:(i + 1) * per] = i + n_before
        e[1, i * per:(i + 1) * per] = torch.arange(i, i + per)
    return e, n_ref + n_before + n_after


def make_features(n_img, feat_dim, hf, wf, seed):
    g = torch.Generator().manual_seed(seed)
    return torch.rand((n_img, feat_dim, hf, wf), generator=g, dtype=torch.float32)


def ray_box_depth(rotmats, tvecs, K, img_size, plane_size):
    n = rotmats.shape[0]
    xs = torch.linspace(0, img_size[1] - 1, plane_size[1])
    ys = torch.linspace(0, img_size[0] - 1, plane_size[0])
    yy, xx = torch.meshgrid(ys, xs, indexing='ij')
    pix = torch.stack((xx, yy, torch.ones_like(xx)), 0).reshape(3, -1).double()
    out = torch.empty((n,) + tuple(plane_size), dtype=torch.float32)
    lo = torch.zeros(3, dtype=torch.float64)
    hi = torch.tensor(ROOM, dtype=torch.float64)
    for i in range(n):
        R = rotmats[i].double()
        c = -(R.T @ tvecs[i].double())
        dirs = R.T @ (torch.inverse(K[i].double()) @ pix)
        t1 = (lo[:, None] - c[:, None]) / dirs
        t2 = (hi[:, None] - c[:, None]) / dirs
        t_exit = torch.maximum(t1, t2).min(dim=0)[0]
        out[i] = t_exit.reshape(plane_size).float()
    return out



def _uniform(g, shape, bound):
    return (torch.rand(shape, generator=g) * 2 - 1) * bound


def _conv_weight(g, shape, fan_in):
    return _uniform(g, shape, 1.0 / math.sqrt(fan_in))


def _norm_stats(g, sd, prefix, c, running=True):
    sd[prefix + '.weight'] = torch.rand(c, generator=g) + 0.5
    sd[prefix + '.bias'] = torch.randn(c, generator=g) * 0.1
    if running:
        sd[prefix + '.running_mean'] = torch.randn(c, generator=g) * 0.1
        sd[prefix + '.running_var'] = torch.rand(c, generator=g) + 0.5


def costregnet_weights(in_channels=32, base=8, seed=0, sharpen=1.0):
    g = torch.Generator().manual_seed(seed)
    sd = {}
    chans = [(in_channels, base), (base, 2 * base), (2 * base, 2 * base), (2 * base, 4 * base),
             (4 * base, 4 * base), (4 * base, 8 * base), (8 * base, 8 * base)]
    for i, (ci, co) in enumerate(chans):
        sd['conv%d.conv.weight' % i] = _conv_weight(g, (co, ci, 3, 3, 3), ci * 27)
        _norm_stats(g, sd, 'conv%d.bn' % i, co)
    for i, (ci, co) in zip((7, 8, 9), [(8 * base, 4 * base), (4 * base, 2 * base), (2 * base, base)]):
        sd['conv%d.deconv.weight' % i] = _conv_weight(g, (ci, co, 3, 3, 3), co * 27)
        _norm_stats(g, sd, 'conv%d.bn' % i, co)
    sd['prob.weight'] = _conv_weight(g, (1, base, 3, 3, 3), base * 27) * sharpen
    sd['prob.bias'] = _uniform(g, (1,), 1.0 / math.sqrt(base * 27))
    return sd


def pointnet_weights(hidden=128, out_dim=64, in_dim=35, seed=1):
    g = torch.Generator().manual_seed(seed)
    sd = {}
    for name, (ci, co) in (('fc_pos', (in_dim, hidden)), ('fc1', (hidden, hidden)),
                           ('fc2', (2 * hidden, hidden)), ('fc3', (2 * hidden, hidden)),
                           ('fc4', (2 * hidden, hidden)), ('fc_out', (hidden, out_dim))):
        b = 1.0 / math.sqrt(ci)
        sd[name + '.weight'] = _uniform(g, (co, ci), b)
        sd[name + '.bias'] = _uniform(g, (co,), b)
    return sd


def sparse_unet_weights(dims=(64, 128, 128), n_groups=(4, 8, 8), n_res=(1, 2, 3), seed=2):
    g = torch.Generator().manual_seed(seed)
    sd = {}

    def res_block(prefix, c):
        for j in (1, 2):
            sd['%s.conv%d.kernel' % (prefix, j)] = _conv_weight(g, (27, c, c), c * 27)
            _norm_stats(g, sd, '%s.n%d.gn' % (prefix, j), c, running=False)

    for i, n in enumerate(n_res):
        for l in range(n):
            res_block('res_down.%d.%d' % (i, l), dims[i])
    for i in range(1, len(dims)):
        sd['down.%d.0.kernel' % (i - 1)] = _conv_weight(g, (27, dims[i - 1], dims[i]), dims[i - 1] * 27)
        _norm_stats(g, sd, 'down.%d.1.gn' % (i - 1), dims[i], running=False)
    rd, rn = dims[::-1], n_res[::-1]
    for i, n in enumerate(rn[1:]):
        for l in range(n):
            res_block('res_up.%d.%d' % (i, l), rd[i + 1])
    for i in range(1, len(rd)):
        sd['up.%d.0.kernel' % (i - 1)] = _conv_weight(g, (27, rd[i - 1], rd[i]), rd[i - 1] * 27)
        _norm_stats(g, sd, 'up.%d.1.gn' % (i - 1), rd[i], running=False)
        sd['feat_adj.%d.0.kernel' % (i - 1)] = _conv_weight(g, (2 * rd[i], rd[i]), 2 * rd[i])
        _norm_stats(g, sd, 'feat_adj.%d.1.gn' % (i - 1), rd[i], running=False)
    return sd


def decoder_weights(in_dim=352, h_dim=128, ksize=3, seed=3, sharpen=1.0):
    g = torch.Generator().manual_seed(seed)
    sd = {}
    for i, ci in enumerate((in_dim, h_dim, h_dim)):
        sd['net.%d.0.weight' % i] = _conv_weight(g, (h_dim, ci, ksize), ci * ksize)
        _norm_stats(g, sd, 'net.%d.1' % i, h_dim)
    sd['net.3.weight'] = _conv_weight(g, (1, h_dim, ksize), h_dim * ksize) * sharpen
    sd['net.3.bias'] = _uniform(g, (1,), 1.0 / math.sqrt(h_dim * ksize))
    return sd


def propagation_weights(in_dim=33, h_dim=32, seed=5):
    g = torch.Generator().manual_seed(seed)
    sd = {}
    widths = [in_dim, h_dim, h_dim, h_dim, 9]
    for i in range(4):
        sd['conv%d.0.weight' % (i + 1)] = _conv_weight(g, (widths[i + 1], widths[i], 3, 3), widths[i] * 9)
        _norm_stats(g, sd, 'conv%d.1' % (i + 1), widths[i + 1])
    return sd


def backbone_weights(feat_dim=32, seed=6):
    from .backbone import FeatureExtractor, FeatureShrinker
    g = torch.Generator().manual_seed(seed)
    out = []
    for mod in (FeatureExtractor(), FeatureShrinker(feat_dim)):
        sd = {}
        for k, v in mod.state_dict().items():
            if k.endswith('num_batches_tracked'):
                continue
            if k.endswith('running_mean'):
                sd[k] = torch.randn(v.shape, generator=g) * 0.1
            elif k.endswith('running_var'):
                sd[k] = torch.rand(v.shape, generator=g) + 0.5
            elif v.dim() == 4:
                fan_in = v.shape[1] * v.shape[2] * v.shape[3]
                sd[k] = _uniform(g, v.shape, math.sqrt(6.0 / fan_in))
            elif k.endswith('bias') and '.fpn.' not in '.' + k:
                sd[k] = torch.randn(v.shape, generator=g) * 0.1
            elif k.endswith('bias'):
                sd[k] = _uniform(g, v.shape, 0.05)
            else:
                sd[k] = torch.rand(v.shape, generator=g) + 0.5
        out.append(sd)
    return tuple(out)


def make_images(n_img, img_size, seed):
    g = torch.Generator().manual_seed(seed)
    low = torch.randn((n_img, 3, img_size[0] // 8, img_size[1] // 8), generator=g)
    return torch.nn.functional.interpolate(low, size=tuple(img_size), mode='bilinear', align_corners=False) \
        + 0.1 * torch.randn((n_img, 3) + tuple(img_size), generator=g)



CONFIGS = {
    'cfg1': dict(img_size=(128, 160), feat_size=(32, 40), depth=(0.5, 0.05, 32),
                 plane_size=(32, 40), window=(1, 1), edge_len=0.08),
    'cfg2': dict(img_size=(256, 320), feat_size=(64, 80), depth=(0.5, 0.05, 96),
                 plane_size=(56, 56), window=(4, 3), edge_len=0.08),
    'cfg3': dict(img_size=(256, 320), feat_size=(64, 80), depth=(0.5, 0.05, 96),
                 plane_size=(56, 56), window=(4, 3), edge_len=0.04),
    'cfg5': dict(img_size=(480, 640), feat_size=(120, 160), depth=(0.5, 0.025, 192),
                 plane_size=(120, 160), window=(5, 5), edge_len=0.02),
}


def make_costvolume_inputs(cfg_name, n_ref, feat_dim=32, seed=None):
    cfg = dict(CONFIGS[cfg_name])
    nb, na = cfg['window']
    edges, n_img = make_edges(n_ref, nb, na)
    if seed is None:
        seed = 1234 + int(cfg_name[-1])
    rotmats, tvecs, K = make_cameras(n_img, cfg['img_size'], seed=seed)
    feat = make_features(n_img, feat_dim, cfg['feat_size'][0], cfg['feat_size'][1], seed)
    cfg.update(feat=feat, rotmats=rotmats, tvecs=tvecs, K=K, edges=edges, n_img=n_img,
               n_ref=n_ref)
    return cfg
```

include/v3d.h:

```cpp
#ifndef V3D_H_
#define V3D_H_

#include <stddef.h>
#include <stdint.h>

#ifdef __cplusplus
extern "C" {
#endif

#define V3D_OK 0
#define V3D_ERR_BAD_SHAPE (-1)
#define V3D_ERR_BAD_ARG (-2)
#define V3D_ERR_WORKSPACE_TOO_SMALL (-3)
#define V3D_ERR_HIP (-4)
#define V3D_ERR_UNSUPPORTED (-5)

#define V3D_PRECISION_SPLIT_BF16 0
#define V3D_PRECISION_FP32 1

int v3d_set_option(const char* name, int value);
int v3d_get_option(const char* name, int* value);

int v3d_version(void);
const char* v3d_last_error(void);

int v3d_timing_enable(int on);
int v3d_timing_collect(int max_entries, char* names_host, int name_stride, float* total_ms_host,
                       int* launches_host);

size_t v3d_edges_csr_workspace_bytes(int n_img, int n_ref);
int v3d_edges_csr(const int64_t* edges, int n_edges, int n_img, int n_ref, int32_t* ref_img, int32_t* edge_ofs,
                  int32_t* edge_src, void* workspace, size_t workspace_bytes, void* stream);
int v3d_edges_csr_status(const void* workspace, size_t workspace_bytes, void* stream);

size_t v3d_psv_workspace_bytes(int n_img, int C, int Hf, int Wf);
int v3d_psv_variance_f32(const float* feat, const float* K, const float* R, const float* t,
                         const int32_t* ref_img, const int32_t* edge_ofs, const int32_t* edge_src,
                         int n_img, int n_ref, int n_edges, int C, int Hf, int Wf, int H, int W,
                         double depth_start, double depth_interval, int D, int h, int w,
                         float* var, void* workspace, size_t workspace_bytes, void* stream);

int v3d_psv_sample_positions_f32(const float* K, const float* R, const float* t, const int32_t* ref_img,
                                 const int32_t* edge_ofs, const int32_t* edge_src, int n_img, int n_ref, int n_edges,
                                 int Hf, int Wf, int H, int W, double depth_start, double depth_interval, int D, int h,
                                 int w, float* pos, float* world, void* workspace, size_t workspace_bytes, void* stream);

int v3d_psv_variance_split(const float* feat, const float* K, const float* R, const float* t,
                         const int32_t* ref_img, const int32_t* edge_ofs, const int32_t* edge_src,
                         int n_img, int n_ref, int n_edges, int C, int Hf, int Wf, int H, int W,
                         double depth_start, double depth_interval, int D, int h, int w,
                         void* var_split, void* workspace, size_t workspace_bytes, void* stream);

int v3d_psv_variance_cl8(const float* feat, const float* K, const float* R, const float* t,
                         const int32_t* ref_img, const int32_t* edge_ofs, const int32_t* edge_src,
                         int n_img, int n_ref, int n_edges, int C, int Hf, int Wf, int H, int W,
                         double depth_start, double depth_interval, int D, int h, int w,
                         float* var_cl8, void* workspace, size_t workspace_bytes, void* stream);

typedef struct v3d_costreg_weights v3d_costreg_weights;

int v3d_costreg_pack(const float* const* conv_weight_host, const float* const* bn_weight_host,
                     const float* const* bn_bias_host, const float* const* bn_mean_host,
                     const float* const* bn_var_host, const float* prob_weight_host,
                     const float* prob_bias_host, int in_channels, int base_channels, float bn_eps,
                     v3d_costreg_weights** out_handle);
void v3d_costreg_free(v3d_costreg_weights* handle);

size_t v3d_costreg_workspace_bytes(const v3d_costreg_weights* handle, int n_ref, int D, int h, int w);
int v3d_costreg_depth_f32(const v3d_costreg_weights* handle, const float* var,
                          const float* depth_vals, int n_ref, int D, int h, int w, float* depth,
                          float* reg, int precision, void* workspace, size_t workspace_bytes, void* stream);
int v3d_costreg_depth_split(const v3d_costreg_weights* handle, const void* var_split,
                          const float* depth_vals, int n_ref, int D, int h, int w, float* depth,
                          float* reg, void* workspace, size_t workspace_bytes, void* stream);
int v3d_costreg_depth_cl8(const v3d_costreg_weights* handle, const void* var_cl8,
                          const float* depth_vals, int n_ref, int D, int h, int w, float* depth,
                          float* reg, void* workspace, size_t workspace_bytes, void* stream);

int v3d_costreg_layer_f32(const v3d_costreg_weights* handle, int layer, const float* in,
                          const float* skip, int n, int Di, int Hi, int Wi, float* out, int precision,
                          void* stream);

size_t v3d_costreg_layer_split_workspace_bytes(int n, int cin, int Di, int Hi, int Wi);
int v3d_costreg_layer_split_f32(const v3d_costreg_weights* handle, int layer, const float* in, const float* skip,
                                int n, int Di, int Hi, int Wi, float* out, void* workspace, size_t workspace_bytes,
                                void* stream);

size_t v3d_backproject_workspace_bytes(int n_img, int C, int Hf, int Wf);
int v3d_backproject_variance_f32(const float* depth, const float* feat, const float* K, const float* R,
                                 const float* t, const int32_t* ref_img, const int32_t* edge_ofs,
                                 const int32_t* edge_src, int n_img, int n_ref, int n_edges, int C,
                                 int Hf, int Wf, int H, int W, int h, int w, double offset, int n_half,
                                 float* pts, float* var, void* workspace, size_t workspace_bytes,
                                 void* stream);

typedef struct v3d_gemm_weights v3d_gemm_weights;
int v3d_gemm_pack(const float* w_host, long long stride_seg, long long stride_co, long long stride_k,
                  int n_seg, int N, int K, const float* scale_host, const float* bias_host,
                  const float* gn_w_host, const float* gn_b_host, v3d_gemm_weights** out_handle);
void v3d_gemm_free(v3d_gemm_weights* handle);
int v3d_gemm_gather_f32(const v3d_gemm_weights* handle, int M, const float* const* seg_src_host,
                        const int32_t* const* seg_idx_host, const int* seg_ld_host, int group_len,
                        int relu_in, int use_gn, float gn_eps, const float* residual, int ld_res,
                        int relu_out, float* pool, const int32_t* pool_idx, int ld_pool, float* out,
                        int ld_out, int precision, void* stream);
int v3d_sparse_conv_f32(const v3d_gemm_weights* handle, int M, const float* src, int ld_src, const int32_t* nbr,
                        long long nbr_stride, int use_gn, float gn_eps, const float* residual, int ld_res, int relu_out,
                        float* out, int ld_out, int precision, void* stream);
int v3d_fill_f32(float* ptr, size_t n, float value, void* stream);
int v3d_pointnet_input_f32(const float* pts, const float* anchor_pts, const float* pts_feat, const int64_t* edge_anchor,
                           const int64_t* edge_pt, int n_edges, int C, float* out, void* stream);

size_t v3d_hash_bytes(int n);
int v3d_hash_build(const int32_t* coords, int n, void* table, size_t table_bytes, void* stream);
int v3d_hash_status(const void* table, int n, void* stream);
int v3d_sparse_neighbors(const void* table, int n_in, const int32_t* out_coords, int n_out, int step,
                         int32_t* nbr, void* stream);
size_t v3d_sparse_interp_workspace_bytes(int n_pts, int n_hyp);
int v3d_sparse_interp_f32(const void* table, int n_in, const float* feats, int C, int tensor_stride,
                          const float* pts, const int64_t* pts_batch, int n_pts, int n_hyp,
                          const float* min_pts, float res, float* out, int ld_out, int col0,
                          void* workspace, size_t workspace_bytes, void* stream);

size_t v3d_segment_csr_workspace_bytes(int n);
int v3d_segment_csr(const int32_t* seg_id, int n, int n_seg, int32_t* perm, int32_t* offsets, void* workspace,
                    size_t workspace_bytes, void* stream);
int v3d_segment_max_f32(const float* src, int ld, const int32_t* perm, const int32_t* offsets, int n_seg, int N, float* out,
                        int ld_out, void* stream);
size_t v3d_sort_unique_workspace_bytes(int n);
int v3d_sort_unique_u64(const uint64_t* keys_in, int n, uint64_t* keys_out, int* n_unique_host,
                        void* workspace, size_t workspace_bytes, void* stream);
int v3d_strided_keys(const int32_t* coords, int n, int tensor_stride, uint64_t* keys_out, void* stream);
int v3d_unpack_coords(const uint64_t* keys, int n, int32_t* coords_out, void* stream);
size_t v3d_voxelize_workspace_bytes(void);
int v3d_voxel_keys(const float* pts, const int64_t* pts_batch, int n, float edge_len, uint64_t* keys_out,
                   void* workspace, size_t workspace_bytes, void* stream);
int v3d_voxelize_status(const void* workspace, size_t workspace_bytes, void* stream);
int v3d_lower_bound_u64(const uint64_t* sorted_unique, int n_unique, const uint64_t* queries, int n,
                        int64_t* index_out, void* stream);
int v3d_voxel_decode(const uint64_t* unique_keys, int n_unique, float edge_len, float half_edge,
                     float* anchor_pts, int32_t* anchor_idx3d, int64_t* anchor_batch, void* workspace,
                     size_t workspace_bytes, void* stream);

int v3d_decoder_head_f32(const float* act, int n_pts, int n_hyp, int C, const float* weight,
                         const float* bias, const float* offset_vals, float* preds, float* expect,
                         void* stream);

typedef struct v3d_propagation_weights v3d_propagation_weights;
int v3d_propagation_pack(const float* const* conv_weight_host, const float* const* bn_weight_host,
                         const float* const* bn_bias_host, const float* const* bn_mean_host,
                         const float* const* bn_var_host, int in_dim, int h_dim, float bn_eps,
                         v3d_propagation_weights** out_handle);
void v3d_propagation_free(v3d_propagation_weights* handle);
int v3d_propagation_up_f32(const v3d_propagation_weights* handle, const float* features, const float* depth_lo, int B, int Cf,
                           int H, int W, int h0, int w0, const int32_t* iy, const int32_t* ix, float* out, int precision, void* stream);

size_t v3d_decoder_fused_workspace_bytes(int n_pts, int n_hyp);
int v3d_decoder_fused_f32(const v3d_gemm_weights* const* layers_host, const float* head_weight, const float* head_bias,
                          const void* const* level_table_host, const int* level_n_host,
                          const float* const* level_feats_host, const int* level_C_host, const int* level_stride_host,
                          const float* const* level_min_pts_host, const float* level_res_host, const float* pts,
                          const int64_t* pts_batch, const float* pts_feat, int c_feat, int n_pts, int n_hyp,
                          const float* offset_vals, float* preds, float* expect, float* depth_inout, void* workspace,
                          size_t workspace_bytes, void* stream);

typedef struct v3d_conv_weights v3d_conv_weights;
int v3d_conv_pack(const float* w_host, const float* bias_host, int cout, int k, v3d_conv_weights** out_handle);
void v3d_conv_free(v3d_conv_weights* handle);
int v3d_conv_nhwc_f32(const v3d_conv_weights* handle, const float* x, int n, int H, int W, int cin, int taps, int relu,
                      int res_mode, const float* res, float* out, void* stream);
int v3d_depthwise_nhwc_f32(const float* x, const float* w, const float* bias, int n, int H, int W, int C, int ksize, int stride,
                           int relu, float* out, void* stream);
int v3d_stem_f32(const float* image, const float* w, const float* bias, int n, int H, int W, float* out, void* stream);
int v3d_nhwc_to_nchw_f32(const float* in, float* out, int n, int C, int HW, void* stream);

typedef struct v3d_irb_weights v3d_irb_weights;
int v3d_irb_pack(const float* w_expand, const float* b_expand, const float* w_dw, const float* b_dw, const float* w_project,
                 const float* b_project, int cin, int mid, int cout, int ksize, int stride, int residual,
                 v3d_irb_weights** out_handle);
void v3d_irb_free(v3d_irb_weights* handle);
int v3d_irb_supported(const v3d_irb_weights* handle, int H, int W);
int v3d_stem_block_pack(const float* w_stem, const float* b_stem, const float* w_dw, const float* b_dw, const float* w_pw,
                        const float* b_pw, v3d_irb_weights** out_handle);
int v3d_stem_block_f32(const v3d_irb_weights* handle, const float* image, int n, int IH, int IW, float* out, void* stream);
size_t v3d_irb_workspace_bytes(const v3d_irb_weights* handle, int n, int H, int W);
int v3d_irb_nhwc_f32(const v3d_irb_weights* handle, const float* x, int n, int H, int W, float* out, void* workspace,
                     size_t workspace_bytes, void* stream);


typedef struct v3d_fpn_weights v3d_fpn_weights;
int v3d_fpn_pack(const float* w_lateral, const float* b_lateral, const float* w_out, const float* b_out, int cin,
                 v3d_fpn_weights** out_handle);
void v3d_fpn_free(v3d_fpn_weights* handle);
int v3d_fpn_level_f32(const v3d_fpn_weights* handle, const float* x, const float* coarse_inner, int n, int H, int W,
                      float* inner_out, float* out, void* stream);

size_t v3d_fusion_workspace_bytes(int n_img, int h, int w);
int v3d_fuse_depths_f32(const float* depths, const float* cams, int n_img, int h, int w, const int32_t* ref_img_host, int n_ref,
                        const int32_t* edge_ofs_host, const int32_t* edge_src_host, double z_thresh, float* pts, int32_t* n_valid,
                        void* workspace, size_t workspace_bytes, void* stream);
int v3d_fusion_compact(const int32_t* n_valid, const float* pts, const void* images, int px_bytes, int n_ref, int h, int w,
                       int n_consistent_thresh, uint8_t* all_valid, int32_t* view_count, int32_t* view_ofs, float* out_pts,
                       void* out_rgb, int32_t* total, void* workspace, size_t workspace_bytes, void* stream);

size_t v3d_cloud_downsample_workspace_bytes(int n);
int v3d_cloud_downsample_f32(const float* pts, const float* attr, int n_attr, int n, const int32_t* n_dev, double voxel_size,
                             float* out_pts, float* out_attr, int32_t* out_count, void* workspace, size_t workspace_bytes,
                             void* stream);
int v3d_cloud_status(const void* workspace, size_t workspace_bytes, int32_t* n_out_host, void* stream);
size_t v3d_nn_workspace_bytes(int n_target, int n_query);
int v3d_nn_query_f32(const float* target, int n_target, const float* query, int n_query, int32_t* idx, float* dist,
                     void* workspace, size_t workspace_bytes, void* stream);
size_t v3d_cloud_metrics_workspace_bytes(void);
int v3d_cloud_metrics_f64(const float* dist_pred, int n_pred, const float* dist_target, int n_target, double threshold,
                          double* out, void* workspace, size_t workspace_bytes, void* stream);

int v3d_tsdf_integrate_f32(float* tsdf, float* weight, float* color, int nx, int ny, int nz, double voxel_size,
                           const float* origin_host, double trunc_margin, const float* projections, const float* depths,
                           const float* images, int n, int h, int w, void* stream);
int v3d_tsdf_normalize_f32(const float* tsdf_sum, const float* weight, const float* color_sum, int n_vox, float* tsdf_out,
                           float* color_out, void* stream);

#define V3D_MESH_MODE_MESH 0
#define V3D_MESH_MODE_POINT_CLOUD 1
size_t v3d_mesh_workspace_bytes(int nx, int ny, int nz);
int v3d_mesh_count_f32(const float* tsdf, int nx, int ny, int nz, int mode, int32_t* counts, void* workspace,
                       size_t workspace_bytes, void* stream);
int v3d_mesh_extract_f32(const float* tsdf, const float* color, int nx, int ny, int nz, double voxel_size,
                         const float* origin_host, int mode, float* verts, uint8_t* colors, int v_cap, int32_t* tris, int f_cap,
                         const void* workspace, size_t workspace_bytes, void* stream);

#ifdef __cplusplus
}
#endif
#endif
```

Before: 18880 depth maps/s.

## Let PSV variance blocks walk several depth chunks per launch block

Adds a WALK variant of the windowed variance kernel. Each block now loops over a contiguous run of depth chunks instead of handling just one. The run length is picked automatically from the grid size so the device still gets enough rounds, and it can be forced through a new psv_walk option. This spreads per-block setup (reference camera, pixel coordinates, source camera loads) over more work and cuts the block count. In exchange each block runs longer, there are fewer blocks for load balancing, and register pressure may rise, so a no-scratch ISA check is added.

```diff
diff --git a/3dvnet_amd/_lib.py b/3dvnet_amd/_lib.py
--- a/3dvnet_amd/_lib.py
+++ b/3dvnet_amd/_lib.py
@@ -30,6 +30,7 @@
     'v3d_timing_collect': (c_int, [c_int, ctypes.c_char_p, c_int, ctypes.POINTER(c_float),
                                    ctypes.POINTER(c_int)]),
     'v3d_psv_workspace_bytes': (c_size_t, [c_int] * 4),
+    'v3d_psv_walk_chunks': (c_int, [c_int] * 4),
     'v3d_psv_variance_f32': (c_int, [c_void_p] * 7 + [c_int] * 8 + [c_double] * 2 + [c_int] * 3 +
                              [c_void_p, c_void_p, c_size_t, c_void_p]),
     'v3d_psv_sample_positions_f32': (c_int, [c_void_p] * 6 + [c_int] * 7 + [c_double] * 2 + [c_int] * 3 +
diff --git a/3dvnet_amd/build.py b/3dvnet_amd/build.py
--- a/3dvnet_amd/build.py
+++ b/3dvnet_amd/build.py
@@ -63,6 +63,7 @@
             isa_check.check_no_scratch(os.path.join(objdir, 'tsdf.o'), 'tsdf_integrate_kernel', strict=strict)
             isa_check.check_no_scratch(os.path.join(objdir, 'cloudmetrics.o'), 'nn_query_kernel', strict=strict)
             isa_check.check_no_scratch(os.path.join(objdir, 'mesh.o'), 'mc_[a-z_]*_kernel', strict=strict)
+            isa_check.check_no_scratch(os.path.join(objdir, 'psv_variance.o'), 'psv_variance_window_kernel', strict=strict)
         finally:
             sys.path.pop(0)
     if force or procs or linked != tag or _stale(LIB, objs):
diff --git a/3dvnet_amd/csrc/api.hip b/3dvnet_amd/csrc/api.hip
--- a/3dvnet_amd/csrc/api.hip
+++ b/3dvnet_amd/csrc/api.hip
@@ -40,7 +40,7 @@
 namespace {
 struct OptDef { const char* name; int def; };
 const OptDef kOptDefs[v3d::kOptCount] = {{"psv_kernel", 0}, {"c12_march", 1}, {"stop_after", 99}, {"gemm_rounds", 1},
-                                         {"gemm_pipe", 1}};
+                                         {"gemm_pipe", 1}, {"psv_walk", 0}};
 std::atomic<int> g_opt[v3d::kOptCount];
 std::atomic<bool> g_opt_init{false};
 void opt_init() {
@@ -66,6 +66,7 @@
     if (!strcmp(name, kOptDefs[i].name)) {
       V3D_REQUIRE(!(i == v3d::kOptGemmRounds || i == v3d::kOptGemmPipe) || value == 0 || value == 1, V3D_ERR_BAD_ARG,
                   "v3d_set_option: %s must be 0 or 1 (got %d)", name, value);
+      V3D_REQUIRE(i != v3d::kOptPsvWalk || value >= 0, V3D_ERR_BAD_ARG, "v3d_set_option: %s must be >= 0 (got %d)", name, value);
       g_opt[i].store(value);
       return V3D_OK;
     }
diff --git a/3dvnet_amd/csrc/psv_variance.hip b/3dvnet_amd/csrc/psv_variance.hip
--- a/3dvnet_amd/csrc/psv_variance.hip
+++ b/3dvnet_amd/csrc/psv_variance.hip
@@ -25,7 +25,8 @@
   int n_img, n_ref, Hf, Wf, H, W, D, h, w, n_ptile;
   double x_step, y_step, z_start, z_step, z_end;
   float rWm1, rHm1;
-  unsigned m_dchunk, m_ptile, m_w;
+  unsigned m_dseg, m_ptile, m_w;
+  int n_dchunk, walk, n_dseg;
 };
 
 
@@ -528,7 +529,7 @@
 #ifndef V3D_PSVW_ABLATE
 #define V3D_PSVW_ABLATE 0
 #endif
-template <bool SPLIT, bool CL8 = false>
+template <bool SPLIT, bool CL8 = false, bool WALK = false>
 __global__ __launch_bounds__(SPLIT ? 64 : 256, V3D_PSV_WAVES) void psv_variance_window_kernel(PsvParams p) {
   static_assert(SPLIT || !CL8, "the channel-last fp32 output uses the single-wave geometry");
   constexpr int C = 32, WPB = SPLIT ? 1 : 4;
@@ -541,6 +542,7 @@
   __shared__ float s_ref_[WPB][24];
   __shared__ float s_P_[WPB][kMaxE][12];
   __shared__ int s_base_[WPB][kMaxE];
+  __shared__ __attribute__((aligned(16))) f32x4 s_xy_[WPB][WALK ? kRPix : 1];
   static_assert(SPLIT || kOutPl * C * (WPB * kRPix + 1) <= WPB * kWinRows * kWinCols * C, "epilogue staging fits the windows");
 
   const int lane = threadIdx.x & 63;
@@ -551,10 +553,11 @@
   float* const s_ref = s_ref_[wv];
   float (*const s_P)[12] = s_P_[wv];
   int* const s_base = s_base_[wv];
-  const int n_dchunk = (p.D + kRDB - 1) / kRDB;
+  f32x4* const s_xy = s_xy_[wv];
   const unsigned b = (unsigned)v3d::xcd_contiguous_block();
-  const unsigned b1 = v3d::udiv_magic(b, (unsigned)n_dchunk, p.m_dchunk), b2 = v3d::udiv_magic(b1, (unsigned)p.n_ptile, p.m_ptile);
-  const int dchunk = (int)(b - b1 * (unsigned)n_dchunk);
+  const unsigned b1 = v3d::udiv_magic(b, (unsigned)p.n_dseg, p.m_dseg), b2 = v3d::udiv_magic(b1, (unsigned)p.n_ptile, p.m_ptile);
+  const int dseg = (int)(b - b1 * (unsigned)p.n_dseg);
+  const int c_begin = WALK ? dseg * p.walk : dseg, c_end = WALK ? min(c_begin + p.walk, p.n_dchunk) : c_begin + 1;
   const int ptile = (int)(b1 - b2 * (unsigned)p.n_ptile) * WPB + wv;
   const int r = (int)b2;
   const int P = p.h * p.w;
@@ -562,12 +565,10 @@
   const int ne = e_end - e_begin;
   const int ref = p.ref_img[r];
   if (lane < 21) s_ref[lane] = p.camp[ref * kCamStride + lane];
-  psv_wave_sync<WPB>();
 
   const int pl1 = lane >> 3, px1 = lane & 7;
   const int gp1 = ptile * kRPix + px1;
-  const int d1 = dchunk * kRDB + pl1;
-  float X, Y, Z;
+  float xf1, yf1;
   {
     int gy, gx;
     if (p.w >= kRPix) {
@@ -580,11 +581,12 @@
     }
     const float xf = (p.w > 1 && gx == p.w - 1) ? (float)(p.W - 1) : (float)((double)gx * p.x_step);
     const float yf = (p.h > 1 && gy == p.h - 1) ? (float)(p.H - 1) : (float)((double)gy * p.y_step);
-    const float z = (d1 == p.D - 1 && p.D > 1) ? (float)p.z_end : (float)(p.z_start + (double)d1 * p.z_step);
-    v3d::world_point(s_ref, xf, yf, z, X, Y, Z);
-  }
-  const bool live1 = gp1 < P && d1 < p.D;
-  const bool all_live = __all(live1);
+    if constexpr (WALK) { if (pl1 == 0) s_xy[px1] = (f32x4){xf, yf, 0.f, 0.f}; }
+    xf1 = xf; yf1 = yf;
+  }
+  psv_wave_sync<WPB>();
+  float X, Y, Z;
+  bool live1, all_live;
   const float Wm1 = (float)(p.W - 1), Hm1 = (float)(p.H - 1);
   const float rWm1 = p.rWm1, rHm1 = p.rHm1;
   const float Wfm1 = (float)(p.Wf - 1), Hfm1 = (float)(p.Hf - 1);
@@ -600,8 +602,6 @@
   const unsigned win_lds = __builtin_amdgcn_readfirstlane(
       (unsigned)(size_t)(__attribute__((address_space(3))) void*)s_win);
   f32x4 acc_s[kRDB], acc_q[kRDB];
-#pragma unroll
-  for (int k = 0; k < kRDB; ++k) acc_s[k] = acc_q[k] = (f32x4){0.f, 0.f, 0.f, 0.f};
 
 #if V3D_PSVW_ABLATE == 1
 #define V3D_PSV_BLEND(pl_, w_) asm volatile("" : : "v"(t00), "v"(t01), "v"(t10), "v"(t11), "v"(w_) : "memory")
@@ -629,8 +629,10 @@
 
   auto load_cams = [&](int e0) __attribute__((always_inline)) {
     const int nload = min(kMaxE, ne - e0) * 12;
+    int lane0 = lane;
+    if constexpr (WALK) asm volatile("" : "+v"(lane0));
 #pragma unroll 1
-    for (int i = lane; i < nload; i += 64) {
+    for (int i = lane0; i < nload; i += 64) {
       const int src = p.edge_src[e_begin + e0 + i / 12];
       s_P[i / 12][i % 12] = p.camp[src * kCamStride + 24 + i % 12];
       if (i % 12 == 0) s_base[i / 12] = src * (p.Hf + 2) * Wp;
@@ -658,167 +660,199 @@
   if (ne > 0) {
     load_cams(0);
     psv_wave_sync<WPB>();
-    project(0, xb, yb, wq);
-  }
-  for (int e = 0; e < ne; ++e) {
+  }
+  const bool cnt_pow2 = (max(ne, 1) & (max(ne, 1) - 1)) == 0;
+  const int cg = lane & 7;
+
+  for (int dchunk = c_begin; dchunk < c_end; ++dchunk) {
+    const int d1 = dchunk * kRDB + pl1;
+    {
+      double z_start = p.z_start, z_end = p.z_end;
+      if constexpr (WALK) asm volatile("" : "+s"(z_start), "+s"(z_end));
+      const float z = (d1 == p.D - 1 && p.D > 1) ? (float)z_end : (float)(z_start + (double)d1 * p.z_step);
+      if constexpr (WALK) {
+        const f32x4 xy = *reinterpret_cast<const f32x4*>(reinterpret_cast<const char*>(s_xy) + cgb);
+        xf1 = xy[0]; yf1 = xy[1];
+      }
+      v3d::world_point(s_ref, xf1, yf1, z, X, Y, Z);
+    }
+    live1 = gp1 < P && d1 < p.D;
+    all_live = __all(live1);
+#pragma unroll
+    for (int k = 0; k < kRDB; ++k) acc_s[k] = acc_q[k] = (f32x4){0.f, 0.f, 0.f, 0.f};
+    if (ne > 0) {
+      if (ne > kMaxE && dchunk != c_begin) {
+        psv_wave_sync<WPB>();
+        load_cams(0);
+        psv_wave_sync<WPB>();
+      }
+      project(0, xb, yb, wq);
+    }
+    for (int e = 0; e < ne; ++e) {
+      psv_wave_sync<WPB>();
+#ifdef V3D_PSV_NOPIPE
+      if (e > 0) {
+        if (e % kMaxE == 0) { load_cams(e); psv_wave_sync<WPB>(); }
+        project(e, xb, yb, wq);
+      }
+#endif
+      int xmin, ymin, ncol, nrow;
+      {
+        const int cc = (yb << 16) | xb;
+        const int ca = __builtin_amdgcn_readlane(cc, 0), cb = __builtin_amdgcn_readlane(cc, 7);
+        const int cd = __builtin_amdgcn_readlane(cc, 56), ce = __builtin_amdgcn_readlane(cc, 63);
+        const int xa = ca & 0xffff, xc = cb & 0xffff, xd = cd & 0xffff, xe = ce & 0xffff;
+        const int ya = ca >> 16, yc = cb >> 16, yd = cd >> 16, ye = ce >> 16;
+        xmin = psv_smin(psv_smin(xa, xc), psv_smin(xd, xe));
+        ymin = psv_smin(psv_smin(ya, yc), psv_smin(yd, ye));
+        ncol = psv_smax(psv_smax(xa, xc), psv_smax(xd, xe)) - xmin + 2 > 8 ? kWinCols : 8;
+        nrow = psv_smin(psv_smax(psv_smax(ya, yc), psv_smax(yd, ye)) - ymin + 2, kWinRows);
+      }
+      const int base_cell = __builtin_amdgcn_readfirstlane(s_base[e % kMaxE]);
+      const unsigned dx = (unsigned)(xb - xmin), dy = (unsigned)(yb - ymin);
+      const bool inwin = dx <= (unsigned)(ncol - 2) && dy <= (unsigned)(nrow - 2);
+      const unsigned so_win = ((dy << 4) | dx) * CB;
+      const unsigned so_ext = ((unsigned)(base_cell + __mul24(yb, Wp) + xb) * CB) | 0x80000000u;
+      const unsigned so = inwin ? so_win : so_ext;
+      s_w[lane] = wq;
+      s_slot[lane] = so;
+      const unsigned prev = (unsigned)__builtin_amdgcn_ds_bpermute(((lane - 8) & 63) * 4, (int)so);
+      const unsigned long long chg = __ballot(lane < 8 || so != prev);
+      {
+        const char* rowp = fb + (size_t)((unsigned)(base_cell + ymin * Wp + xmin) * CB);
+        unsigned dst = win_lds;
+        asm volatile("s_nop 4" ::: "memory");
+#pragma unroll 1
+        for (int rr = 0; rr < (V3D_PSVW_ABLATE == 3 ? 0 : nrow); ++rr) {
+          unsigned keep;
+          asm volatile("s_mov_b32 %0, m0\n\ts_mov_b32 m0, %3\n\ts_nop 0\n\tglobal_load_lds_dwordx4 %1, %2\n\ts_mov_b32 m0, %0"
+                       : "=&s"(keep) : "v"(lane16), "s"(rowp), "s"(dst) : "memory");
+          if (ncol > 8)
+            asm volatile("s_mov_b32 %0, m0\n\ts_mov_b32 m0, %3\n\ts_nop 0\n\tglobal_load_lds_dwordx4 %1, %2 offset:1024\n\ts_mov_b32 m0, %0"
+                         : "=&s"(keep) : "v"(lane16), "s"(rowp), "s"(dst) : "memory");
+          rowp += (size_t)Wp * CB;
+          dst += kWinCols * CB;
+        }
+      }
+#ifndef V3D_PSV_NOPIPE
+      if (e + 1 < ne) {
+        if ((e + 1) % kMaxE == 0) {
+          psv_wave_sync<WPB>();
+          load_cams(e + 1);
+          psv_wave_sync<WPB>();
+        }
+        project(e + 1, xb, yb, wq);
+      }
+#endif
+      asm volatile("s_waitcnt vmcnt(0) lgkmcnt(0)" ::: "memory");
+      psv_wave_sync<WPB>();
+      f32x4 t00, t01, t10, t11;
+      f32x4 wn = s_w[gpx];
+      unsigned sn = s_slot[gpx];
+#pragma unroll
+      for (int pl = 0; pl < kRDB; ++pl) {
+        const f32x4 w = wn;
+        const unsigned so_pl = sn;
+        if (pl + 1 < kRDB) {
+          wn = s_w[(pl + 1) * kRPix + gpx];
+          sn = s_slot[(pl + 1) * kRPix + gpx];
+        }
+        if (((chg >> (8 * pl)) & 0xffull) && (V3D_PSVW_ABLATE != 2 || (pl == 0 && e == 0))) {
+          if (V3D_PSVW_ABLATE != 6 && (int)so_pl < 0) {
+            const unsigned b00 = so_pl & 0x7fffffffu;
+            t00 = *reinterpret_cast<const f32x4*>(fb + (size_t)(b00 + cgb));
+            t01 = *reinterpret_cast<const f32x4*>(fb + (size_t)(b00 + cgb) + CB);
+            t10 = *reinterpret_cast<const f32x4*>(fb + (size_t)(b00 + rowb));
+            t11 = *reinterpret_cast<const f32x4*>(fb + (size_t)(b00 + rowb) + CB);
+          } else {
+            const char* a = wb + (so_pl + cgb);
+            t00 = *reinterpret_cast<const f32x4*>(a);
+            t01 = *reinterpret_cast<const f32x4*>(a + CB);
+            t10 = *reinterpret_cast<const f32x4*>(a + kWinCols * CB);
+            t11 = *reinterpret_cast<const f32x4*>(a + kWinCols * CB + CB);
+          }
+        }
+        V3D_PSV_BLEND(pl, w);
+      }
+    }
+
     psv_wave_sync<WPB>();
-#ifdef V3D_PSV_NOPIPE
-    if (e > 0) {
-      if (e % kMaxE == 0) { load_cams(e); psv_wave_sync<WPB>(); }
-      project(e, xb, yb, wq);
-    }
-#endif
-    int xmin, ymin, ncol, nrow;
-    {
-      const int cc = (yb << 16) | xb;
-      const int ca = __builtin_amdgcn_readlane(cc, 0), cb = __builtin_amdgcn_readlane(cc, 7);
-      const int cd = __builtin_amdgcn_readlane(cc, 56), ce = __builtin_amdgcn_readlane(cc, 63);
-      const int xa = ca & 0xffff, xc = cb & 0xffff, xd = cd & 0xffff, xe = ce & 0xffff;
-      const int ya = ca >> 16, yc = cb >> 16, yd = cd >> 16, ye = ce >> 16;
-      xmin = psv_smin(psv_smin(xa, xc), psv_smin(xd, xe));
-      ymin = psv_smin(psv_smin(ya, yc), psv_smin(yd, ye));
-      ncol = psv_smax(psv_smax(xa, xc), psv_smax(xd, xe)) - xmin + 2 > 8 ? kWinCols : 8;
-      nrow = psv_smin(psv_smax(psv_smax(ya, yc), psv_smax(yd, ye)) - ymin + 2, kWinRows);
-    }
-    const int base_cell = __builtin_amdgcn_readfirstlane(s_base[e % kMaxE]);
-    const unsigned dx = (unsigned)(xb - xmin), dy = (unsigned)(yb - ymin);
-    const bool inwin = dx <= (unsigned)(ncol - 2) && dy <= (unsigned)(nrow - 2);
-    const unsigned so_win = ((dy << 4) | dx) * CB;
-    const unsigned so_ext = ((unsigned)(base_cell + __mul24(yb, Wp) + xb) * CB) | 0x80000000u;
-    const unsigned so = inwin ? so_win : so_ext;
-    s_w[lane] = wq;
-    s_slot[lane] = so;
-    const unsigned prev = (unsigned)__builtin_amdgcn_ds_bpermute(((lane - 8) & 63) * 4, (int)so);
-    const unsigned long long chg = __ballot(lane < 8 || so != prev);
-    {
-      const char* rowp = fb + (size_t)((unsigned)(base_cell + ymin * Wp + xmin) * CB);
-      unsigned dst = win_lds;
-      asm volatile("s_nop 4" ::: "memory");
-#pragma unroll 1
-      for (int rr = 0; rr < (V3D_PSVW_ABLATE == 3 ? 0 : nrow); ++rr) {
-        unsigned keep;
-        asm volatile("s_mov_b32 %0, m0\n\ts_mov_b32 m0, %3\n\ts_nop 0\n\tglobal_load_lds_dwordx4 %1, %2\n\ts_mov_b32 m0, %0"
-                     : "=&s"(keep) : "v"(lane16), "s"(rowp), "s"(dst) : "memory");
-        if (ncol > 8)
-          asm volatile("s_mov_b32 %0, m0\n\ts_mov_b32 m0, %3\n\ts_nop 0\n\tglobal_load_lds_dwordx4 %1, %2 offset:1024\n\ts_mov_b32 m0, %0"
-                       : "=&s"(keep) : "v"(lane16), "s"(rowp), "s"(dst) : "memory");
-        rowp += (size_t)Wp * CB;
-        dst += kWinCols * CB;
-      }
-    }
-#ifndef V3D_PSV_NOPIPE
-    if (e + 1 < ne) {
-      if ((e + 1) % kMaxE == 0) {
-        psv_wave_sync<WPB>();
-        load_cams(e + 1);
-        psv_wave_sync<WPB>();
-      }
-      project(e + 1, xb, yb, wq);
-    }
-#endif
-    asm volatile("s_waitcnt vmcnt(0) lgkmcnt(0)" ::: "memory");
-    psv_wave_sync<WPB>();
-    f32x4 t00, t01, t10, t11;
-    f32x4 wn = s_w[gpx];
-    unsigned sn = s_slot[gpx];
-#pragma unroll
-    for (int pl = 0; pl < kRDB; ++pl) {
-      const f32x4 w = wn;
-      const unsigned so_pl = sn;
-      if (pl + 1 < kRDB) {
-        wn = s_w[(pl + 1) * kRPix + gpx];
-        sn = s_slot[(pl + 1) * kRPix + gpx];
-      }
-      if (((chg >> (8 * pl)) & 0xffull) && (V3D_PSVW_ABLATE != 2 || (pl == 0 && e == 0))) {
-        if (V3D_PSVW_ABLATE != 6 && (int)so_pl < 0) {
-          const unsigned b00 = so_pl & 0x7fffffffu;
-          t00 = *reinterpret_cast<const f32x4*>(fb + (size_t)(b00 + cgb));
-          t01 = *reinterpret_cast<const f32x4*>(fb + (size_t)(b00 + cgb) + CB);
-          t10 = *reinterpret_cast<const f32x4*>(fb + (size_t)(b00 + rowb));
-          t11 = *reinterpret_cast<const f32x4*>(fb + (size_t)(b00 + rowb) + CB);
-        } else {
-          const char* a = wb + (so_pl + cgb);
-          t00 = *reinterpret_cast<const f32x4*>(a);
-          t01 = *reinterpret_cast<const f32x4*>(a + CB);
-          t10 = *reinterpret_cast<const f32x4*>(a + kWinCols * CB);
-          t11 = *reinterpret_cast<const f32x4*>(a + kWinCols * CB + CB);
-        }
-      }
-      V3D_PSV_BLEND(pl, w);
-    }
-  }
-#undef V3D_PSV_BLEND
-
-  psv_wave_sync<WPB>();
-  const float cnt = (float)max(ne, 1);
-  const bool cnt_pow2 = (max(ne, 1) & (max(ne, 1) - 1)) == 0;
-  const float cnt_inv = 1.f / cnt;
-  const int cg = lane & 7;
-  if constexpr (SPLIT) {
-    const int chunk = cg >> 1, half = cg & 1;
-    u32x4* const out = reinterpret_cast<u32x4*>(p.var);
-    const int gp = ptile * kRPix + gpx;
-    u32x4* const obase = out + (((size_t)r * 8 + chunk * 2 + half) * p.D + (size_t)dchunk * kRDB) * P + gp;
+    int tid_o = (int)threadIdx.x;
+    if constexpr (WALK) asm volatile("" : "+v"(tid_o));
+    int ne_o = ne;
+    if constexpr (WALK) asm volatile("" : "+s"(ne_o));
+    const float cnt = (float)max(ne_o, 1);
+    const float cnt_inv = 1.f / cnt;
+    if constexpr (SPLIT) {
+      const int chunk = cg >> 1, half = cg & 1;
+      u32x4* const out = reinterpret_cast<u32x4*>(p.var);
+      const int gp = ptile * kRPix + (tid_o >> 3);
+      u32x4* const obase = WALK ? out + ((size_t)r * 8 * p.D + (size_t)dchunk * kRDB) * P +
+                                      ((unsigned)(chunk * 2 + half) * (unsigned)(p.D * P) + (unsigned)gp)
+                                : out + (((size_t)r * 8 + chunk * 2 + half) * p.D + (size_t)dchunk * kRDB) * P + gp;
 #define V3D_PSV_EMIT(MEAN)                                                                                              \
-  _Pragma("unroll") for (int pl = 0; pl < kRDB; ++pl) {                                                                 \
-    float v[4];                                                                                                         \
-    _Pragma("unroll") for (int k = 0; k < 4; ++k) {                                                                     \
-      const float avg = MEAN(acc_s[pl][k]);                                                                             \
-      const float avg_sq = MEAN(acc_q[pl][k]);                                                                          \
-      v[k] = v3d::sub_rn(avg_sq, v3d::mul_rn(avg, avg));                                             \
-    }                                                                                                                   \
-    const int d = dchunk * kRDB + pl;                                                                                   \
-    if constexpr (CL8) {                                                                                                \
+    _Pragma("unroll") for (int pl = 0; pl < kRDB; ++pl) {                                                               \
+      float v[4];                                                                                                       \
+      _Pragma("unroll") for (int k = 0; k < 4; ++k) {                                                                   \
+        const float avg = MEAN(acc_s[pl][k]);                                                                           \
+        const float avg_sq = MEAN(acc_q[pl][k]);                                                                        \
+        v[k] = v3d::sub_rn(avg_sq, v3d::mul_rn(avg, avg));                                           \
+      }                                                                                                                 \
+      const int d = dchunk * kRDB + pl;                                                                                 \
+      if constexpr (CL8) {                                                                                              \
                \
-      const u32x4 slot = {__float_as_uint(v[0]), __float_as_uint(v[1]), __float_as_uint(v[2]), __float_as_uint(v[3])};  \
-      if (gp < P && d < p.D)                                                                                            \
+        const u32x4 slot = {__float_as_uint(v[0]), __float_as_uint(v[1]), __float_as_uint(v[2]), __float_as_uint(v[3])};\
+        if (gp < P && d < p.D)                                                                                          \
+          __builtin_nontemporal_store(slot, obase + (size_t)pl * (unsigned)P);                                           \
+      } else {                                                                                                          \
+      const unsigned h01 = pack_bf16x2(v[0], v[1]), h23 = pack_bf16x2(v[2], v[3]);                                      \
+      const unsigned l01 = pack_bf16x2(v[0] - __uint_as_float(h01 << 16), v[1] - __uint_as_float(h01 & 0xffff0000u));   \
+      const unsigned l23 = pack_bf16x2(v[2] - __uint_as_float(h23 << 16), v[3] - __uint_as_float(h23 & 0xffff0000u));   \
+      const unsigned s0 = half ? h01 : l01, s1 = half ? h23 : l23;                     \
+      const unsigned r0 = (unsigned)__builtin_amdgcn_mov_dpp((int)s0, 0xB1, 0xf, 0xf, true);    \
+      const unsigned r1 = (unsigned)__builtin_amdgcn_mov_dpp((int)s1, 0xB1, 0xf, 0xf, true);                            \
+      const u32x4 slot = half ? (u32x4){r0, r1, l01, l23} : (u32x4){h01, h23, r0, r1};                                  \
+      if (gp < P && d < p.D && (V3D_PSVW_ABLATE != 5 || slot[0] == 0x12345u))                                           \
         __builtin_nontemporal_store(slot, obase + (size_t)pl * (unsigned)P);                                             \
-    } else {                                                                                                            \
-    const unsigned h01 = pack_bf16x2(v[0], v[1]), h23 = pack_bf16x2(v[2], v[3]);                                        \
-    const unsigned l01 = pack_bf16x2(v[0] - __uint_as_float(h01 << 16), v[1] - __uint_as_float(h01 & 0xffff0000u));     \
-    const unsigned l23 = pack_bf16x2(v[2] - __uint_as_float(h23 << 16), v[3] - __uint_as_float(h23 & 0xffff0000u));     \
-    const unsigned s0 = half ? h01 : l01, s1 = half ? h23 : l23;                       \
-    const unsigned r0 = (unsigned)__builtin_amdgcn_mov_dpp((int)s0, 0xB1, 0xf, 0xf, true);      \
-    const unsigned r1 = (unsigned)__builtin_amdgcn_mov_dpp((int)s1, 0xB1, 0xf, 0xf, true);                              \
-    const u32x4 slot = half ? (u32x4){r0, r1, l01, l23} : (u32x4){h01, h23, r0, r1};                                    \
-    if (gp < P && d < p.D && (V3D_PSVW_ABLATE != 5 || slot[0] == 0x12345u))                                             \
-      __builtin_nontemporal_store(slot, obase + (size_t)pl * (unsigned)P);                                               \
-    }                                                                                                                   \
-  }
+      }                                                                                                                 \
+    }
 #define V3D_MEAN_MUL(x) ((x) * cnt_inv)
 #define V3D_MEAN_DIV(x) __builtin_amdgcn_div_fixupf(v3d::div_uniform((x), cnt, cnt_inv), cnt, (x))
-    if (cnt_pow2) { V3D_PSV_EMIT(V3D_MEAN_MUL) } else { V3D_PSV_EMIT(V3D_MEAN_DIV) }
+      if (cnt_pow2) { V3D_PSV_EMIT(V3D_MEAN_MUL) } else { V3D_PSV_EMIT(V3D_MEAN_DIV) }
 #undef V3D_PSV_EMIT
 #undef V3D_MEAN_MUL
 #undef V3D_MEAN_DIV
-  } else {
-    constexpr int NPX = WPB * kRPix;
-    float (*const s_out)[C][NPX + 1] = reinterpret_cast<float (*)[C][NPX + 1]>(&s_win_[0][0]);
-    auto mean = [&](float x) __attribute__((always_inline)) {
-      return cnt_pow2 ? x * cnt_inv : __builtin_amdgcn_div_fixupf(v3d::div_uniform(x, cnt, cnt_inv), cnt, x);
-    };
-    const int gp0 = (ptile - wv) * kRPix;
-#pragma unroll
-    for (int round = 0; round < kRDB / kOutPl; ++round) {
-      __syncthreads();
-#pragma unroll
-      for (int q = 0; q < kOutPl; ++q) {
-        const int pl = round * kOutPl + q;
-#pragma unroll
-        for (int k = 0; k < 4; ++k) {
-          const float avg = mean(acc_s[pl][k]);
-          const float avg_sq = mean(acc_q[pl][k]);
-          s_out[q][cg * 4 + k][wv * kRPix + gpx] = v3d::sub_rn(avg_sq, v3d::mul_rn(avg, avg));
-        }
-      }
-      __syncthreads();
-      for (int i = threadIdx.x; i < kOutPl * C * NPX; i += 64 * WPB) {
-        const int q = i / (C * NPX), c = (i / NPX) % C, px = i % NPX;
-        const int gp = gp0 + px, d = dchunk * kRDB + round * kOutPl + q;
-        if (gp < P && d < p.D) __builtin_nontemporal_store(s_out[q][c][px], &p.var[(((size_t)r * C + c) * p.D + d) * P + gp]);
-      }
-    }
-  }
+    } else {
+      constexpr int NPX = WPB * kRPix;
+      float (*const s_out)[C][NPX + 1] = reinterpret_cast<float (*)[C][NPX + 1]>(&s_win_[0][0]);
+      auto mean = [&](float x) __attribute__((always_inline)) {
+        return cnt_pow2 ? x * cnt_inv : __builtin_amdgcn_div_fixupf(v3d::div_uniform(x, cnt, cnt_inv), cnt, x);
+      };
+      const int gp0 = (ptile - wv) * kRPix;
+#pragma unroll
+      for (int round = 0; round < kRDB / kOutPl; ++round) {
+        __syncthreads();
+#pragma unroll
+        for (int q = 0; q < kOutPl; ++q) {
+          const int pl = round * kOutPl + q;
+#pragma unroll
+          for (int k = 0; k < 4; ++k) {
+            const float avg = mean(acc_s[pl][k]);
+            const float avg_sq = mean(acc_q[pl][k]);
+            s_out[q][cg * 4 + k][wv * kRPix + gpx] = v3d::sub_rn(avg_sq, v3d::mul_rn(avg, avg));
+          }
+        }
+        __syncthreads();
+        for (int i = tid_o; i < kOutPl * C * NPX; i += 64 * WPB) {
+          const int q = i / (C * NPX), c = (i / NPX) % C, px = i % NPX;
+          const int gp = gp0 + px, d = dchunk * kRDB + round * kOutPl + q;
+          if (gp < P && d < p.D) __builtin_nontemporal_store(s_out[q][c][px], &p.var[(((size_t)r * C + c) * p.D + d) * P + gp]);
+        }
+      }
+      if (WALK && dchunk + 1 < c_end) __syncthreads();
+    }
+  }
+#undef V3D_PSV_BLEND
 }
 
 __global__ __launch_bounds__(256) void psv_positions_kernel(PsvParams p, float* __restrict__ pos, float* __restrict__ world) {
@@ -866,6 +900,20 @@
 
 extern "C" size_t v3d_psv_workspace_bytes(int n_img, int C, int Hf, int Wf) {
   return v3d::align_up(psv_feat_bytes(n_img, C, Hf, Wf), 256) + v3d::align_up((size_t)n_img * kCamStride * sizeof(float), 256);
+}
+
+static int psv_walk_chunks(int forced, int n_dchunk, int n_ref, int n_ptile) {
+  constexpr long long kResident = 256 * 4 * V3D_PSV_WAVES, kMinRounds = 16;
+  long long walk = forced > 0 ? forced : (long long)n_ref * n_dchunk * n_ptile / (kMinRounds * kResident);
+  walk = walk < 1 ? 1 : walk > n_dchunk ? n_dchunk : walk;
+  if (forced > 0) return (int)walk;
+  const long long n_dseg = (n_dchunk + walk - 1) / walk;
+  return (int)((n_dchunk + n_dseg - 1) / n_dseg);
+}
+
+extern "C" int v3d_psv_walk_chunks(int n_ref, int D, int h, int w) {
+  V3D_REQUIRE(n_ref > 0 && D > 0 && h > 0 && w > 0, V3D_ERR_BAD_SHAPE, "v3d_psv_walk_chunks: bad shape");
+  return psv_walk_chunks(v3d::option(v3d::kOptPsvWalk), (D + kRDB - 1) / kRDB, n_ref, (h * w + kRPix - 1) / kRPix);
 }
 
 static int psv_variance_impl(int mode, const float* feat, const float* K, const float* R,
@@ -933,26 +981,36 @@
       const bool no_window = reuse_env || psv_feat_bytes(n_img, C, Hf, Wf) >= ((size_t)1 << 31);
       V3D_REQUIRE(!cl8 || !no_window, V3D_ERR_UNSUPPORTED,
                   "v3d_psv_variance_cl8: only the window kernel writes this layout (feature maps < 2 GB, no developer switch)");
+      unsigned wblocks = 0;
       {
         const unsigned ndc = (unsigned)((D + kRDB - 1) / kRDB);
         const unsigned npt = (unsigned)(split || cl8 ? p.n_ptile : (p.n_ptile + 3) / 4);
-        const unsigned long long nblk = (unsigned long long)n_ref * ndc * npt;
+        p.n_dchunk = (int)ndc;
+        p.walk = psv_walk_chunks(v3d::option(v3d::kOptPsvWalk), (int)ndc, n_ref, p.n_ptile);
+        if ((split || cl8) && 8ull * D * h * w >= (1ull << 32)) p.walk = 1;
+        p.n_dseg = ((int)ndc + p.walk - 1) / p.walk;
+        const unsigned long long nblk = (unsigned long long)n_ref * p.n_dseg * npt;
+        wblocks = (unsigned)nblk;
         p.rWm1 = (float)(1.0 / (double)(W - 1));
         p.rHm1 = (float)(1.0 / (double)(H - 1));
-        p.m_dchunk = v3d::magic_u32(nblk, ndc);
-        p.m_ptile = v3d::magic_u32(nblk / ndc + 1, npt);
+        p.m_dseg = v3d::magic_u32(nblk, (unsigned)p.n_dseg);
+        p.m_ptile = v3d::magic_u32(nblk / p.n_dseg + 1, npt);
         p.m_w = v3d::magic_u32((unsigned long long)h * w + 4 * kRPix, (unsigned)w);
       }
+      const bool walk = p.walk > 1;
       if (cl8) {
-        psv_variance_window_kernel<true, true><<<(unsigned)rblocks, 64, 0, s>>>(p);
+        if (walk) psv_variance_window_kernel<true, true, true><<<wblocks, 64, 0, s>>>(p);
+        else psv_variance_window_kernel<true, true, false><<<wblocks, 64, 0, s>>>(p);
       } else if (split) {
         if (no_window) psv_variance_reuse_kernel<true><<<(unsigned)rblocks, 64, 0, s>>>(p);
-        else psv_variance_window_kernel<true><<<(unsigned)rblocks, 64, 0, s>>>(p);
+        else if (walk) psv_variance_window_kernel<true, false, true><<<wblocks, 64, 0, s>>>(p);
+        else psv_variance_window_kernel<true, false, false><<<wblocks, 64, 0, s>>>(p);
       } else {
         p.n_ptile = (p.n_ptile + 3) / 4;
         const long long fblocks = (long long)n_ref * ((D + kRDB - 1) / kRDB) * p.n_ptile;
         if (no_window) psv_variance_reuse_kernel<false><<<(unsigned)fblocks, 256, 0, s>>>(p);
-        else psv_variance_window_kernel<false><<<(unsigned)fblocks, 256, 0, s>>>(p);
+        else if (walk) psv_variance_window_kernel<false, false, true><<<wblocks, 256, 0, s>>>(p);
+        else psv_variance_window_kernel<false, false, false><<<wblocks, 256, 0, s>>>(p);
       }
     } else if (cl8) {
       return v3d::fail(V3D_ERR_UNSUPPORTED, "v3d_psv_variance_cl8: C=%d unsupported (32) / option psv_kernel = 2", C);
diff --git a/3dvnet_amd/csrc/v3d_common.h b/3dvnet_amd/csrc/v3d_common.h
--- a/3dvnet_amd/csrc/v3d_common.h
+++ b/3dvnet_amd/csrc/v3d_common.h
@@ -50,6 +50,7 @@
   kOptStopAfter,
   kOptGemmRounds,
   kOptGemmPipe,
+  kOptPsvWalk,
   kOptCount
 };
 int option(Option o);
diff --git a/3dvnet_amd/synthetic.py b/3dvnet_amd/synthetic.py
--- a/3dvnet_amd/synthetic.py
+++ b/3dvnet_amd/synthetic.py
@@ -230,3 +230,14 @@
     cfg.update(feat=feat, rotmats=rotmats, tvecs=tvecs, K=K, edges=edges, n_img=n_img,
                n_ref=n_ref)
     return cfg
+
+
+def make_exotic_cameras(img_size=(64, 80), seed=9):
+    R, tv, K = make_cameras(6, img_size, seed=seed)
+    K = K.clone(); K[1, 0, 0] *= 3.0; K[1, 1, 1] *= 3.0
+    c, s_ = math.cos(math.pi / 2), math.sin(math.pi / 2)
+    roll = torch.tensor([[c, -s_, 0.0], [s_, c, 0.0], [0.0, 0.0, 1.0]])
+    R = R.clone(); tv = tv.clone()
+    R[2] = roll @ R[2]; tv[2] = roll @ tv[2]
+    tv[3] = tv[3] + torch.tensor([0.8, 0.0, 0.0])
+    return R, tv, K
diff --git a/include/v3d.h b/include/v3d.h
--- a/include/v3d.h
+++ b/include/v3d.h
@@ -34,6 +34,7 @@
 int v3d_edges_csr_status(const void* workspace, size_t workspace_bytes, void* stream);
 
 size_t v3d_psv_workspace_bytes(int n_img, int C, int Hf, int Wf);
+int v3d_psv_walk_chunks(int n_ref, int D, int h, int w);
 int v3d_psv_variance_f32(const float* feat, const float* K, const float* R, const float* t,
                          const int32_t* ref_img, const int32_t* edge_ofs, const int32_t* edge_src,
                          int n_img, int n_ref, int n_edges, int C, int Hf, int Wf, int H, int W,
```

After: 19270 depth maps/s (median of 6 runs). +2.1%, better.
